# usamec/GAML

Measured on AMD Instinct MI355X. Metric: reads_per_sec_scored, higher is better.
Workload: dtype f64; 1 GPU; cfg3: 5 Mbp, 50x 2x150 paired, insert 300+-30; 833333 pairs in all, whole true genome as 1-2 walks, 8 rotating path sets, window cache warm; pairs_total=833333, pairs_per_gpu=833333, genome_bp=5000000, parallelism=reads sharded over 1 GPU(s)

## Files before the change

### gaml_amd/api.py

```python
from __future__ import annotations

import ctypes as C
import importlib.util
import os
import sys

import numpy as np

_HERE = os.path.dirname(os.path.abspath(__file__))
FLAVOUR = os.environ.get("GAML_HIP_FLAVOUR", "release")
LIB_PATH = os.environ.get("GAML_HIP_LIB") or os.path.join(_HERE, "libgaml_hip_dev.so" if FLAVOUR == "dev" else "libgaml_hip.so")

OK, EINVAL, ENODEVICE, EHIP, ESTATE = 0, -1, -2, -3, -4

_i32p = np.ctypeslib.ndpointer(np.int32, flags="C_CONTIGUOUS")
_i64p = np.ctypeslib.ndpointer(np.int64, flags="C_CONTIGUOUS")
_f64p = np.ctypeslib.ndpointer(np.float64, flags="C_CONTIGUOUS")
_u8p = np.ctypeslib.ndpointer(np.uint8, flags="C_CONTIGUOUS")

ALIGMENT = np.dtype([("position", np.int32), ("edit_dist", np.int32), ("read_id", np.int32), ("orientation", np.int32)])
PACBIO_ALIGMENT = np.dtype([("position", np.int32), ("position_end", np.int32), ("read_id", np.int32), ("pad_", np.int32),
                            ("logprob", np.float64)])


# ... 123 lines not shown
    L.gaml_hip_eval_coverage_finish_async.argtypes = [vp, C.c_int32, vp, C.c_int32, C.c_int32, vp]
    L.gaml_hip_eval_pacbio_pending.argtypes = [vp]
    L.gaml_hip_eval_pacbio_pending.restype = C.c_int32
    L.gaml_hip_eval_pacbio_intervals.argtypes = [vp, C.c_int32]
    L.gaml_hip_eval_pacbio_intervals.restype = C.c_int64
    L.gaml_hip_eval_pacbio_export_async.argtypes = [vp, C.c_int32, vp, C.c_int64, vp]
    L.gaml_hip_eval_pacbio_finish_async.argtypes = [vp, C.c_int32, vp, C.c_int64, C.c_int32, vp]
    L.gaml_hip_num_readsets.argtypes = [vp]
    L.gaml_hip_readset_kind.argtypes = [vp, C.c_int]
    L.gaml_hip_readset_reads.argtypes = [vp, C.c_int]
    L.gaml_hip_readset_reads.restype = C.c_int64
    L.gaml_hip_num_nodes.argtypes = [vp]
    L.gaml_hip_node_len.argtypes = [vp, C.c_int32]
    L.gaml_hip_read_probs.argtypes = [vp, C.c_int, _f64p, C.c_int64]
    L.gaml_hip_bad_bases.argtypes = [vp, C.c_int, C.POINTER(C.c_int64)]
    L.gaml_hip_window_count.argtypes = [vp, C.c_int, C.c_int]
    L.gaml_hip_window_count.restype = C.c_int64
    L.gaml_hip_window_records.argtypes = [vp, C.c_int, C.c_int, _i32p, C.c_int32, vp, C.c_int64]
    L.gaml_hip_window_records.restype = C.c_int64
    L.gaml_hip_align_window.argtypes = [vp, C.c_int, C.c_int, _i32p, C.c_int32]
    L.gaml_hip_align_window.restype = C.c_int64
    if hasattr(L, "gaml_hip_debug_prepare"):
        L.gaml_hip_debug_prepare.argtypes = [vp, _i32p, _i64p, C.c_int32]
    if hasattr(L, "gaml_hip_debug_occurrences"):
        L.gaml_hip_debug_occurrences.argtypes = [vp, C.c_int, C.c_int, _i32p, C.c_int64]
    if hasattr(L, "gaml_hip_debug_occurrences"):
        L.gaml_hip_debug_occurrences.restype = C.c_int64
    if hasattr(L, "gaml_hip_debug_table_occurrences"):
        L.gaml_hip_debug_table_occurrences.argtypes = [vp, C.c_int, C.c_int, _i32p, C.c_int64, _i64p]
    if hasattr(L, "gaml_hip_debug_table_occurrences"):
        L.gaml_hip_debug_table_occurrences.restype = C.c_int64
    if hasattr(L, "gaml_hip_debug_cov_layout"):
        L.gaml_hip_debug_cov_layout.argtypes = [vp, C.c_int, vp, C.c_int32, vp, vp, vp, C.c_int32, vp, C.c_int32, vp]
        L.gaml_hip_debug_cov_layout.restype = C.c_int32
    if hasattr(L, "gaml_hip_debug_window_walk"):
        L.gaml_hip_debug_window_walk.argtypes = [vp, C.c_int, C.c_int, C.c_int32, _i32p, C.c_int32]
    for new, old in (("gaml_hip_pair_classes", "gaml_hip_debug_class_counts"), ("gaml_hip_last_phases", "gaml_hip_debug_profile"),
                     ("gaml_hip_table_stats", "gaml_hip_debug_table_stats")):
        if not hasattr(L, new) and hasattr(L, old):
            setattr(L, new, getattr(L, old))
    L.gaml_hip_pair_classes.argtypes = [vp, C.c_int, _i64p]
    if hasattr(L, "gaml_hip_debug_fold_check"):
        L.gaml_hip_debug_fold_check.argtypes = [vp, C.c_int, _i64p]
    if hasattr(L, "gaml_hip_debug_radix_sort"):
        L.gaml_hip_debug_radix_sort.argtypes = [vp, C.c_void_p, C.c_void_p, C.c_int64, C.c_int, C.c_int, C.c_void_p]
    if hasattr(L, "gaml_hip_debug_tables_check"):
        L.gaml_hip_debug_tables_check.argtypes = [vp, C.c_int, _i64p]
    if hasattr(L, "gaml_hip_debug_static_check"):
        L.gaml_hip_debug_static_check.argtypes = [vp, C.c_int, _i64p]
    if hasattr(L, "gaml_hip_debug_set_knob"):
        L.gaml_hip_debug_set_knob.argtypes = [vp, C.c_int, C.c_int]
    if hasattr(L, "gaml_hip_debug_occ_route"):
        L.gaml_hip_debug_occ_route.argtypes = [vp, C.c_int, _i64p]
    if hasattr(L, "gaml_hip_debug_occ_check"):
        L.gaml_hip_debug_occ_check.argtypes = [vp, C.c_int, _i64p]
    if hasattr(L, "gaml_hip_debug_batch_bad_bases"):
        L.gaml_hip_debug_batch_bad_bases.argtypes = [vp, C.c_int, C.c_void_p, C.c_int32]
        L.gaml_hip_debug_batch_bad_bases.restype = C.c_int32
    if hasattr(L, "gaml_hip_shm_exchange_open"):
        L.gaml_hip_shm_exchange_open.argtypes = [vp, C.c_char_p, C.c_int32, C.c_int32, C.c_int32]
        L.gaml_hip_shm_allreduce_sum.argtypes = [vp, C.c_void_p, C.c_int32]
        L.gaml_hip_shm_exchange_close.argtypes = [vp, C.c_int32]
    if hasattr(L, "gaml_hip_fetch_async"):
        L.gaml_hip_fetch_async.argtypes = [vp, C.c_void_p, C.c_int32, C.c_void_p]
        L.gaml_hip_fetch_wait.argtypes = [vp, C.c_void_p, C.c_int32]
    if hasattr(L, "gaml_hip_advice_build"):
        L.gaml_hip_advice_build.argtypes = [vp, C.c_int, C.c_int32]
        L.gaml_hip_advice_index.argtypes = [vp, C.c_int, C.c_void_p, C.c_void_p, C.c_int64]
        L.gaml_hip_advice_index.restype = C.c_int64
        L.gaml_hip_advice_candidates.argtypes = [vp, C.c_int, _i32p, C.c_int32, _i32p, C.c_int32, C.c_int32, C.c_void_p, C.c_int64]
        L.gaml_hip_advice_candidates.restype = C.c_int64
    if hasattr(L, "gaml_hip_gap_profile"):
        L.gaml_hip_gap_profile.argtypes = [vp, _i32p, _i64p, C.c_int32, C.c_int32, C.c_int32, C.c_void_p, C.c_int32, C.c_void_p, C.c_void_p, C.c_void_p]
        L.gaml_hip_fix_gap_length.argtypes = [vp, _i32p, _i64p, C.c_int32, C.c_int32, C.c_int32, C.POINTER(C.c_int32), C.c_void_p, C.c_void_p,
                                              C.c_int32, C.POINTER(C.c_int32)]
        L.gaml_hip_gap_stats.argtypes = [vp, _i64p]
    if hasattr(L, "gaml_hip_debug_timeline"):
        L.gaml_hip_debug_timeline.argtypes = [vp, C.c_int, C.c_void_p, C.c_int64]
    L.gaml_hip_last_phases.argtypes = [vp, _f64p]
    L.gaml_hip_table_stats.argtypes = [vp, C.c_int, _i64p]
    L.gaml_hip_aligner_stats.argtypes = [vp, C.POINTER(C.c_int64), C.POINTER(C.c_int64), C.POINTER(C.c_double)]
    L.gaml_hip_aligner_stages.argtypes = [vp, _f64p]
    L.gaml_hip_last_timing.argtypes = [vp, _f64p]
    L.gaml_hip_set_event_timing.argtypes = [vp, C.c_int]
    L.gaml_hip_kernel_stats.argtypes = [vp, C.c_int, C.POINTER(C.c_int64), C.POINTER(C.c_double), C.POINTER(C.c_double)]
    return L


_lib = _load()

def lib():
    return _lib


def version() -> str:
    return _lib.gaml_hip_version().decode()


class FlatPaths:

    def __init__(self, paths):
        self.flat, self.offs = _flat(paths)
        self.n = len(paths)
        self.flat_ptr, self.offs_ptr = self.flat.ctypes.data, self.offs.ctypes.data

    def __len__(self):
# ... 475 lines not shown
        return {"full_rebuilds": int(out[0]), "delta_updates": int(out[1]), "dirty_pairs": int(out[2]), "worker_rebuilds": int(out[3]), "side_stream_rebuilds": int(out[3]),
                "batches_patched": int(out[4]), "batches_full": int(out[5]), "records_left_out": [int(out[6]), int(out[7])], "delta_records_left_out": int(out[8]),
                "static_index_pairs": int(out[9])}

    def aligner_stats(self):
        w, k, us = C.c_int64(), C.c_int64(), C.c_double()
        _lib.gaml_hip_aligner_stats(self._h, C.byref(w), C.byref(k), C.byref(us))
        return {"windows": w.value, "candidates": k.value, "us": us.value}

    def aligner_stages(self):
        out = np.zeros(6, np.float64)
        self._check(_lib.gaml_hip_aligner_stages(self._h, out))
        return {"strings_upload": out[0], "spans_candidates": out[1], "extension": out[2], "hits_d2h": out[3], "sort_file": out[4], "batches": int(out[5])}

    def last_phases(self):
        out = np.zeros(8, np.float64)
        _lib.gaml_hip_last_phases(self._h, out)
        return out

    def debug_timeline(self, rs: int, cap_waves: int = 1 << 16) -> np.ndarray:
        out = np.zeros((cap_waves, 8), np.uint64)
        n = self._check(_lib.gaml_hip_debug_timeline(self._h, rs, out.ctypes.data, cap_waves))
        return out[:n]

    def debug_set_knob(self, knob, value):
        self._check(_lib.gaml_hip_debug_set_knob(self._h, knob, value))

    def debug_fold_check(self, rs):
        out = np.zeros(6, np.int64)
        self._check(_lib.gaml_hip_debug_fold_check(self._h, rs, out))
        return {"records_left_out": [int(out[0]), int(out[1])], "compact_pairs": [int(out[2]), int(out[3])], "records_checked": int(out[4]),
                "violations": int(out[5])}

    def debug_radix_sort(self, keys, vals=None, begin_bit=0, end_bit=64, running_max=False):
        k = np.ascontiguousarray(keys, np.uint64).copy()
        v = None if vals is None else np.ascontiguousarray(vals, np.uint64).copy()
        m = np.zeros(len(k), np.uint64) if running_max else None
        self._check(_lib.gaml_hip_debug_radix_sort(self._h, k.ctypes.data, None if v is None else v.ctypes.data, len(k), begin_bit, end_bit,
                                                   None if m is None else m.ctypes.data))
        return k, v, m

    def debug_static_check(self, rs):
        out = np.zeros(8, np.int64)
        self._check(_lib.gaml_hip_debug_static_check(self._h, rs, out))
        return {"static_pairs": int(out[0]), "other_pairs": int(out[1]), "violations": int(out[2]), "no_record": int(out[3]),
                "different_windows": int(out[4]), "orientation": int(out[5]), "distance": int(out[6]), "edits_or_code": int(out[7])}

    def debug_occ_route(self, rs):
        out = np.zeros(6, np.int64)
        self._check(_lib.gaml_hip_debug_occ_route(self._h, rs, out))
        return {"device": int(out[0]), "host": int(out[1]), "fallbacks": int(out[2]), "compactions": int(out[3]),
                "pool_entries": int(out[4]), "shared_combinations": int(out[5])}

    def debug_occ_check(self, rs):
        out = np.zeros(4, np.int64)
        rc = _lib.gaml_hip_debug_occ_check(self._h, rs, out)
        res = {"compared": int(out[0]), "present": int(out[1]), "mismatches": int(out[2]), "lists": int(out[3])}
        if rc != 0 and res["compared"] == 0:
            self._check(rc)
        return res

    def debug_batch_bad_bases(self, rs):
        n = self._check(_lib.gaml_hip_debug_batch_bad_bases(self._h, rs, None, 0))
        out = np.zeros(max(1, n), np.int64)
        self._check(_lib.gaml_hip_debug_batch_bad_bases(self._h, rs, out.ctypes.data, n))
        return out[:n].tolist()

    def debug_tables_check(self, rs):
        out = np.zeros(8, np.int64)
        rc = _lib.gaml_hip_debug_tables_check(self._h, rs, out)
        res = {"pairs": int(out[0]), "compact": int(out[1]), "static": int(out[2]), "two": int(out[3]), "four": int(out[4]), "more": int(out[5]),
               "compared": int(out[6]), "mismatches": int(out[7])}
        if rc != 0 and res["compared"] == 0:
            self._check(rc)
        return res

    def debug_block_partials(self, rs, set_index=0):
        sums, zeros, lay = np.zeros(8192, np.float64), np.zeros(8192, np.int32), np.zeros(8, np.int32)
        _lib.gaml_hip_debug_block_partials.argtypes = [C.c_void_p, C.c_int, C.c_int32, _f64p, _i32p, C.c_int32, _i32p]
        n = _lib.gaml_hip_debug_block_partials(self._h, rs, set_index, sums, zeros, 8192, lay)
        return sums[:max(n, 0)].copy(), zeros[:max(n, 0)].copy(), lay.tolist()

    def pair_classes(self, rs):
        out = np.zeros(4, np.int64)
        self._check(_lib.gaml_hip_pair_classes(self._h, rs, out))
        return out

    debug_table_stats, debug_profile, debug_class_counts = table_stats, last_phases, pair_classes

    def last_timing(self):
        out = np.zeros(3, np.float64)
        _lib.gaml_hip_last_timing(self._h, out)
        return {"host_us": out[0], "device_wall_us": out[1], "kernel_us": out[2]}

    def set_event_timing(self, on):
        _lib.gaml_hip_set_event_timing(self._h, int(on))

    def kernel_stats(self, reset=False):
        n, us, b = C.c_int64(), C.c_double(), C.c_double()
        _lib.gaml_hip_kernel_stats(self._h, 1 if reset else 0, C.byref(n), C.byref(us), C.byref(b))
        return {"launches": n.value, "device_us": us.value, "algo_bytes": b.value}


def debug_sam_band(sam_line: str, total_len: int):
    raw = sam_line.encode()
    f = np.zeros(10, np.int32); r0 = np.zeros(1, np.int32)
# ... 20 lines not shown
```

### gaml_amd/csrc/ctx.hip.h

```cpp
#pragma once
#include <hip/hip_runtime.h>
#include <hip/hip_ext.h>
#include "radix_sort.hip.h"

#include <algorithm>
#include <atomic>
#include <fcntl.h>
#include <sys/mman.h>
#include <unistd.h>
#include <chrono>
#include <climits>
#include <limits>
#include <cmath>
#include <cstdio>
#include <cstdlib>
#include <cstring>
#include <immintrin.h>
#include <memory>
#include <set>
#include <string>
#include <thread>
#include <vector>

#include "aligner.hip.h"
// ... 229 lines not shown
  PairInfo pt;
  MateDev dev[2];
  TableDev tab;
  TableRebuild rebuild;
  BuildScratch scratch;
  BuildPlan build_plan;
  int64_t async_rebuilds = 0, retired_windows = 0, eval_count = 0;
  DevBuf lcode, len_combo_dev, combo_tabs, memo;
  int memo_codes = 0;
  bool statics_uploaded = false, kernels_warm = false, prereserved = false;
  DevBuf dl_slot, dl_spill, dl_rec[2], sp_rng[2], sp_rec[2], sp_slot, dstate;
  DevBuf dl_bins, dl_bin_count, dl_blk_tot, dl_wlist, dl_stamps;
  PinBuf h_dstate;
  size_t delta_cap = 0, cap_spill = 0, cap_sprec = 0;
  int64_t nd_est = 0, ns_est = 0;
  bool spill_may_grow = false;
  int dl_seq = 0;
  int64_t full_rebuilds = 0, delta_updates = 0;
  int quiet_calls = 0;
  int64_t delta_left_out = 0, delta_left_out_base = 0;
  bool compact_requested = false;
  PinBuf h_timeline; int timeline_waves = 0;
  PinBuf h_part_sum, h_part_zero;
  size_t host_part_stride = 0;
  int last_total_blocks = 0, last_sets = 1;
  int last_blocks[8] = {0, 0, 0, 0, 0, 0, 0, 0};
  bool last_host_partials = false;
  DevBuf probs, tabs, cov_bits, bad;
  DevBuf cov_multi;
  size_t cov_multi_used = 0;
  PinBuf h_bad;
  std::vector<int64_t> batch_bad;
  Arena arena;
  struct Persist {
    void* dev = nullptr; size_t bytes = 0;
    size_t cap_w[2] = {0, 0}, cap_lo[2] = {0, 0}, cap_m[2] = {0, 0};
    size_t off_tfloor = 0, off_occ[2] = {0, 0}, off_lo[2] = {0, 0}, off_m[2] = {0, 0};
    size_t cap_cov = 0, off_cov = 0;
    bool valid = false;
    size_t last_bytes = 0;
    void release() { if (dev) (void)hipFree(dev); dev = nullptr; bytes = 0; valid = false; }
  } persist;
  struct OccDev {
    DevBuf pool[2];
    size_t pool_cap[2] = {0, 0}, pool_used[2] = {0, 0};
    uint32_t pool_gen = 1;
    PinBuf stage;
    DevBuf tab[2][2], list[2][2];
    DevBuf stamp[2];
    size_t cap_w = 0, cap_list = 0;
    int32_t list_n[2][2] = {{0, 0}, {0, 0}};
    uint32_t serial = 0;
    PinBuf dup;
    bool taken = false;
    bool check_dup = false;
    bool image_stale = false;
    std::vector<std::vector<uint64_t>> shared;
    size_t shared_next = 0;
    std::vector<uint64_t> key;
    int64_t dev_calls = 0, host_calls = 0, fallbacks = 0, compactions = 0;
    void release() {
      for (int mt = 0; mt < 2; mt++) {
        pool[mt].release(); stamp[mt].release();
        for (int k = 0; k < 2; k++) { tab[mt][k].release(); list[mt][k].release(); }
      }
      stage.release(); dup.release();
    }
  } occdev;
  int64_t batches_patched = 0, batches_full = 0;
  size_t batch_slack = 0;
  hipEvent_t ev_tables = nullptr, ev_ovf = nullptr;
  PairedPlanner planner;
  OccImage image[2];
  std::vector<Occ> scratch_occ[2];
  Reducer red;
  Staging stage_pool;
  std::vector<double> ins_tab, floor_tab, logfloor_tab, covthr_tab;
  bool floor_positive = true;
  bool tabs_uploaded = false;
  int64_t last_bad_bases = 0;
  AdviceDev adv;
};

struct SingleSet {
  gaml_single_cfg cfg;
  ShortMate mate;
  ReadMajor rm;
  MateDev dev;
  DevBuf lens, probs, tabs, occ_arena;
  std::vector<Occ> last_occ;
  Reducer red;
  std::vector<double> floor_tab, logfloor_tab;
  bool tabs_uploaded = false;
  Staging stage;
};

struct DpDev {
  DevBuf path, jobs, ops, scratch, out, dbg;
  void release() { path.release(); jobs.release(); ops.release(); scratch.release(); out.release(); dbg.release(); }
};

struct PbSweepDev {
  DevBuf iv_off, iv;
  std::vector<int32_t> iv_off_host;
  uint64_t generation = ~0ull;
  DevBuf in, all;
  DevBuf key_begin, key_end, pos, key_begin_s, key_end_s, pos_s, end_max, tmp, bad;
  Staging stage;
  void release() {
    iv_off.release(); iv.release(); in.release(); all.release(); key_begin.release(); key_end.release(); pos.release();
    key_begin_s.release(); key_end_s.release(); pos_s.release(); end_max.release(); tmp.release(); bad.release();
    for (int k = 0; k < kRing; k++) { stage.host[k].release(); if (stage.done[k]) (void)hipEventDestroy(stage.done[k]); stage.done[k] = nullptr; stage.armed[k] = false; }
  }
};

struct PacbioSet {
// ... 8 lines not shown
  int64_t misses = 0;
  DevBuf d_lens, rec_off, rec_walk, rec_logp, walk_count, logprobs;
  Reducer red;
  int64_t last_bad_bases = 0;
  Staging stage;
  PbSweepDev sweep;
  bool have_reads = false;
  std::string bases;
  std::vector<int64_t> base_off;
  std::unordered_map<std::string, int32_t> name_id;
  DevBuf d_bases;
  DpDev dp;
  bool bases_uploaded = false;
  double dp_stats[8] = {0, 0, 0, 0, 0, 0, 0, 0};
};

struct PairedPrep {
  int64_t assembled_records = 0;
  std::vector<int32_t> slot_base, path_base, start_off, starts;
  int32_t total_bits = 0, n_paths = 0;
  bool general = false;
};

struct SetRef { int kind, idx; };

}
}

using namespace gaml;
using namespace gaml::detail;

struct gaml_hip_ctx {
  gaml::MultiState* multi = nullptr;
  gaml::CommState* comm = nullptr;
  int device = -1;
  DevBuf warm_buf; bool general_warm = false;
  AlnJob aln_job[2];
  hipStream_t stream = nullptr;
  hipStream_t aux_stream = nullptr;
  GraphStore g;
  bool have_graph = false;
  std::vector<std::unique_ptr<SingleSet>> singles;
  std::vector<std::unique_ptr<PairedSet>> paireds;
  std::vector<std::unique_ptr<PacbioSet>> pacbios;
  std::vector<SetRef> handles;
  int32_t rank = 0, world = 1;
  bool multi_shard = false;
  AlignScratch aln_scratch;
  AlignSmall aln_small[2];
  int64_t aln_windows = 0, aln_candidates = 0;
  double aln_us = 0;
  double aln_stage_us[5] = {0, 0, 0, 0, 0};
  int64_t aln_batches = 0;
  int knobs[24] = {0};
  bool direct_write = false;
  int32_t peers = 1;
  std::string err;
  bool event_timing = false;
  int event_every = 1;
  int64_t event_tick = 0;
  std::vector<std::pair<hipEvent_t, hipEvent_t>> ev_pool;
  std::vector<uint64_t> ev_call;
  uint64_t eval_serial = 0;
  size_t ev_used = 0;
  double t_host_us = 0, t_dev_wall_us = 0, t_kernel_us = 0;
  int64_t stat_launches = 0;
  double stat_device_us = 0, stat_algo_bytes = 0;
  DevBuf packed;
  PinBuf packed_host;
  char* shm_base = nullptr; size_t shm_bytes = 0; int shm_rank = 0, shm_world = 0, shm_cap = 0; unsigned long long shm_step = 0; std::string shm_name;
  PinBuf fetch_host;
  unsigned long long fetch_seq = 0;
  hipStream_t fetch_stream = nullptr;
  DevBuf batch_dev;
  PinBuf batch_host;
  int64_t gap_stats[4] = {0, 0, 0, 0};
  std::vector<int32_t> gap_flat;
  std::vector<int64_t> gap_offs;
  bool pending_open = false;
  std::vector<Walk> pending_paths;
  bool pending_paths_valid = false;
  int32_t pending_total_len = 0;
  std::vector<std::unique_ptr<PairedPrep>> pending_prep;
  double pending_host_us = 0;
  double prof[8] = {0, 0, 0, 0, 0, 0, 0, 0};
  bool used_default_stream = false;
  double* status_dst = nullptr; double status_a = 0, status_b = 0; bool status_done = false;
  bool host_results = false;
  bool occ_route = false;
  bool defer_cov = false;
  struct PendingCov { int paired_idx; CovArgs args; double* out4; };
  std::vector<PendingCov> pending_cov;
  struct PendingPacbio {
    int pacbio_idx;
    double* out4;
    int32_t n_paths;
    int64_t n_node, n_own;
  };
  std::vector<PendingPacbio> pending_pb;
};
```

### gaml_amd/csrc/debug_api.hip.h

```cpp
#pragma once

int gaml_hip_debug_prepare(gaml_hip_ctx* c, const int32_t* flat, const int64_t* offs, int32_t n_paths) {
  if (!c || n_paths < 0 || (n_paths > 0 && (!flat || !offs))) return fail(c, GAML_HIP_EINVAL, "bad arguments");
  if (c->multi) {
    for (int k = 0; k < gaml::multi_num_shards(c->multi); k++)
      if (int e = gaml_hip_debug_prepare(gaml::multi_shard(c->multi, k), flat, offs, n_paths)) return fail(c, e, gaml_hip_last_error(gaml::multi_shard(c->multi, k)));
    return GAML_HIP_OK;
  }
  if (!c->have_graph) return fail(c, GAML_HIP_ESTATE, "no graph set");
  std::vector<Walk> paths = unflatten(flat, offs, n_paths);
  for (auto& h : scoring_order(c)) {
    if (h.kind == 0) { std::vector<Occ> occs; prepare_single_host(c, *c->singles[h.idx], paths, occs); }
    else if (h.kind == 1) {
      PairedPrep p;
      PairedSet& ps = *c->paireds[h.idx];
      if (int e = prepare_paired_structure(c, ps, flat, offs, n_paths)) return e;
      if (int e = align_pending_pair(c, ps)) return e;
      if (int e = prepare_paired_tables_host(c, ps, p)) return e;
    }
  }
  if (c->peers == 1) {
    for (ShortMate* m : filter_mates(c)) m->unsynced.clear();
  }
  return GAML_HIP_OK;
// ... 28 lines not shown
  for (Occ& o : v) { auto it = pos.find(o.path); o.path = it == pos.end() ? -1 : it->second; }
  std::sort(v.begin(), v.end(), [](const Occ& a, const Occ& b) { return a.path != b.path ? a.path < b.path : (a.rank != b.rank ? a.rank < b.rank : a.wid < b.wid); });
  for (int64_t i = 0; i < (int64_t)v.size() && i < cap; i++) {
    const Occ& o = v[(size_t)i];
    out5[5 * i] = o.wid; out5[5 * i + 1] = o.shift; out5[5 * i + 2] = o.min_pos; out5[5 * i + 3] = o.path; out5[5 * i + 4] = o.rank;
  }
  return (int64_t)v.size();
}

int32_t gaml_hip_debug_cov_layout(gaml_hip_ctx* c, int rs, int32_t* slot_base, int32_t cap_slots, int32_t* path_base, int32_t* start_off, int32_t* slots,
                                   int32_t cap_paths, int32_t* starts, int32_t cap_starts, int32_t* counts4) {
  MULTI_SHARD0(c);
  if (!c || rs < 0 || rs >= (int)c->handles.size() || c->handles[rs].kind != 1) return -1;
  PairedSet& ps = *c->paireds[c->handles[rs].idx];
  if (!(ps.cfg.penalty_constant > 0) || ps.planner.full_calls + ps.planner.incremental_calls == 0) return -1;
  struct { std::vector<int32_t> slot_base, path_base, start_off, starts, slots; } L;
  {
    PairedPrep p;
    paired_cov_build(ps, true, p);
    L.slot_base.swap(p.slot_base); L.path_base.swap(p.path_base); L.start_off.swap(p.start_off); L.starts.swap(p.starts);
    L.slots = ps.planner.slots();
  }
  const int32_t n = (int32_t)L.slots.size();
  if (counts4) { counts4[0] = (int32_t)L.slot_base.size(); counts4[1] = n; counts4[2] = (int32_t)L.starts.size(); counts4[3] = L.path_base.back(); }
  for (int32_t k = 0; k < (int32_t)L.slot_base.size() && k < cap_slots; k++) slot_base[k] = L.slot_base[k];
  for (int32_t k = 0; k <= n && k <= cap_paths && cap_paths > 0; k++) { path_base[k] = L.path_base[k]; start_off[k] = L.start_off[k]; }
  for (int32_t k = 0; k < n && k < cap_paths; k++) slots[k] = L.slots[k];
  for (int32_t k = 0; k < (int32_t)L.starts.size() && k < cap_starts; k++) starts[k] = L.starts[k];
  return n;
}

int32_t gaml_hip_debug_window_walk(gaml_hip_ctx* c, int rs, int mate, int32_t wid, int32_t* out, int32_t cap) {
  MULTI_SHARD0(c);
  ShortMate* m = mate_of(c, rs, mate);
  if (!m || wid < 0 || wid >= (int32_t)m->win_walk.size()) return -1;
  const Walk& w = *m->win_walk[wid];
  for (int32_t i = 0; i < (int32_t)w.size() && i < cap; i++) out[i] = w[i];
  return (int32_t)w.size();
}



int gaml_hip_debug_timeline(gaml_hip_ctx* c, int rs, unsigned long long* out, int64_t cap_waves) {
  MULTI_SHARD0(c);
  if (!c || rs < 0 || rs >= (int)c->handles.size() || c->handles[rs].kind != 1 || !out) return fail(c, GAML_HIP_EINVAL, "bad arguments");
  PairedSet& s = *c->paireds[c->handles[rs].idx];
  if (!s.h_timeline.p) return 0;
  const int64_t n = std::min<int64_t>(cap_waves, s.timeline_waves);
  memcpy(out, s.h_timeline.p, (size_t)n * 8 * sizeof(unsigned long long));
  return (int)n;
}

int gaml_hip_debug_set_knob(gaml_hip_ctx* c, int knob, int value) {
  if (!c || knob < 0 || knob >= 24) return GAML_HIP_EINVAL;
  if (c->multi) { for (int k = 0; k < gaml::multi_num_shards(c->multi); k++) gaml::multi_shard(c->multi, k)->knobs[knob] = value; return GAML_HIP_OK; }
  c->knobs[knob] = value;
  return GAML_HIP_OK;
}


static void paired_base_records(const PairTables& pt, int32_t slot, int mt, std::vector<RecQuad>& out) {
  const int64_t n0s = pt.class_count[0];
  if (slot < n0s) {
    const uint64_t r = pt.rec8[mt][slot];
    if (r != kNoRec8) out.push_back(RecQuad{(int32_t)(r & 0xffffff), (int32_t)((r >> 24) & 0xfffffff), (int32_t)((r >> 52) & 63) | ((int32_t)((r >> 58) & 1) << 8), 0});
  } else {
    const RecQuad& f = pt.rm[mt].first[slot - n0s];
    if (f.wid >= 0) {
      const int cnt1 = 1 + (int)((uint32_t)f.flags >> 9);
      for (int q = 0; q < cnt1; q++) { RecQuad r = q == 0 ? f : pt.rm[mt].extra[f.link + q - 1]; r.flags &= 0x1ff; r.link = 0; out.push_back(r); }
    }
  }
}

int gaml_hip_debug_fold_check(gaml_hip_ctx* c, int rs, int64_t* out6) {
  MULTI_SHARD0(c);
  if (!c || rs < 0 || rs >= (int)c->handles.size() || c->handles[rs].kind != 1 || !out6) return fail(c, GAML_HIP_EINVAL, "bad arguments");
  PairedSet& s = *c->paireds[c->handles[rs].idx];
  for (int mt = 0; mt < 2; mt++) for (const Window& w : s.mate[mt].wins) if (w.first < 0 && w.count > 0) return fail(c, GAML_HIP_ESTATE, "host-only check: some windows' records exist in the device pool only (use gaml_hip_debug_tables_check)");
  PairTables with, without;
  build_pair_tables(s.mate[0], s.mate[1], with, true);
  build_pair_tables(s.mate[0], s.mate[1], without, false);
  int64_t checked = 0, bad = 0;
  const int64_t n = s.mate[0].n_local();
  std::vector<RecQuad> a, b;
  for (int mt = 0; mt < 2; mt++) {
    const ShortMate& m = s.mate[mt];
    for (int64_t read = 0; read < n; read++) {
      a.clear(); b.clear();
      paired_base_records(with, with.slot_of_read[read], mt, a);
      paired_base_records(without, without.slot_of_read[read], mt, b);
      size_t ia = 0;
      for (size_t ib = 0; ib < b.size(); ib++) {
        checked++;
        const RecQuad& r = b[ib];
        if (ia < a.size() && a[ia].wid == r.wid && a[ia].pos == r.pos && a[ia].flags == r.flags) { ia++; continue; }
        const Window& j = m.wins[r.wid];
        bool ok = false;
        if (j.head >= 0) {
          auto it = m.solo_of_node.find(j.head);
          if (it != m.solo_of_node.end() && m.wins[it->second].active)
            for (size_t q = 0; q < b.size(); q++) ok = ok || (b[q].wid == it->second && b[q].pos == r.pos);
        }
        bad += !ok;
      }
      bad += ia != a.size();
    }
// ... 122 lines not shown
    for (Window& w : hm[mt].wins) if (w.dfirst < 0) { w.count = 0; }
  }
  PairTables pt;
  build_pair_tables(hm[0], hm[1], pt, KNOB(c, 16) != 1, paired_static_ins_n(c, s));
  const int64_t n = s.mate[0].n_local();
  int64_t compared = 0, bad = 0;
  auto fetch = [&](const DevBuf& d, size_t bytes, std::vector<char>& out) -> int {
    out.resize(bytes);
    if (bytes) HIP_TRY(c, hipMemcpy(out.data(), d.p, bytes, hipMemcpyDeviceToHost));
    return 0;
  };
  auto cmp = [&](const DevBuf& d, const void* host, size_t bytes, size_t elem, const char* what) -> int {
    std::vector<char> v;
    if (int e = fetch(d, bytes, v)) return e;
    int64_t b0 = bad;
    for (size_t k = 0; k < bytes / elem; k++) { compared++; if (memcmp(v.data() + k * elem, (const char*)host + k * elem, elem) != 0) bad++; }
    if (bad != b0 && getenv("GAML_HIP_TRACE_HOST")) fprintf(stderr, "tables_check: %s differs in %lld of %zu entries\n", what, (long long)(bad - b0), bytes / elem);
    return 0;
  };
  for (int k = 0; k < 4; k++) { compared++; bad += T.class_count[k] != pt.class_count[k]; }
  compared++; bad += T.n0a != pt.n0a;
  if (bad == 0) {
    const int64_t n0 = pt.class_count[0], n16 = n - n0;
    if (int e = cmp(T.slot_of_read, pt.slot_of_read.data(), (size_t)n * 4, 4, "slot_of_read")) return e;
    if (int e = cmp(T.read_of_slot, pt.read_of_slot.data(), (size_t)n * 4, 4, "read_of_slot")) return e;
    for (int mt = 0; mt < 2; mt++) {
      if (int e = cmp(T.rec8[mt], pt.rec8[mt].data(), (size_t)n0 * 8, 8, "rec8")) return e;
      if (int e = cmp(T.first[mt], pt.rm[mt].first.data(), (size_t)n16 * 16, 16, "first")) return e;
      if (int e = cmp(T.extra[mt], pt.rm[mt].extra.data(), pt.rm[mt].extra.size() * 16, 16, "extra")) return e;
      if (int e = cmp(T.inl[mt], pt.inl[mt].data(), pt.inl[mt].size() * 16, 16, "inl")) return e;
      compared++; bad += T.extras[mt] != (int64_t)pt.rm[mt].extra.size();
      compared++; bad += T.dropped[mt] != pt.dropped_records[mt];
    }
    if (int e = cmp(T.len_code, pt.len_code.data(), (size_t)n0, 1, "len_code")) return e;
    if (int e = cmp(T.static_idx, pt.static_idx.data(), (size_t)pt.n0a * 4, 4, "static_idx")) return e;
    if (int e = cmp(T.len12, pt.len12.data(), (size_t)n16 * 4, 4, "len12")) return e;
    compared++; bad += pt.len_combo != s.pt.len_combo;
  }
  out8[0] = n; out8[1] = T.class_count[0]; out8[2] = T.n0a; out8[3] = T.class_count[1]; out8[4] = T.class_count[2]; out8[5] = T.class_count[3];
  out8[6] = compared; out8[7] = bad;
  T.release();
  return bad ? fail(c, GAML_HIP_ESTATE, "record tables: the device build differs from the host restatement") : GAML_HIP_OK;
}

int gaml_hip_debug_occ_route(gaml_hip_ctx* c, int rs, int64_t* out6) {
  MULTI_SHARD0(c);
  if (!c || !out6 || rs < 0 || rs >= (int)c->handles.size() || c->handles[rs].kind != 1) return fail(c, GAML_HIP_EINVAL, "bad arguments");
  const PairedSet::OccDev& D = c->paireds[c->handles[rs].idx]->occdev;
  out6[0] = D.dev_calls; out6[1] = D.host_calls; out6[2] = D.fallbacks; out6[3] = D.compactions;
  out6[4] = (int64_t)(D.pool_used[0] + D.pool_used[1]); out6[5] = (int64_t)D.shared.size();
  return GAML_HIP_OK;
}

int gaml_hip_debug_occ_check(gaml_hip_ctx* c, int rs, int64_t* out4) {
  MULTI_SHARD0(c);
  if (!c || !out4 || rs < 0 || rs >= (int)c->handles.size() || c->handles[rs].kind != 1) return fail(c, GAML_HIP_EINVAL, "bad arguments");
  PairedSet& ps = *c->paireds[c->handles[rs].idx];
  const PairedSet::OccDev& D = ps.occdev;
  out4[0] = out4[1] = out4[2] = out4[3] = 0;
  if (!D.image_stale) return GAML_HIP_OK;
  HIP_TRY(c, hipSetDevice(c->device));
  HIP_TRY(c, hipStreamSynchronize(c->stream));
  const PlanView& v = ps.planner.view();
  for (int mt = 0; mt < 2; mt++) {
    OccImage im;
    im.build(ps.mate[mt].wins.size(), v, mt);
    const size_t n = im.occ12.size();
    std::vector<Occ12> dev(n);
    if (n) HIP_TRY(c, hipMemcpy(dev.data(), occdev_table(ps, mt), n * sizeof(Occ12), hipMemcpyDeviceToHost));
    for (size_t w = 0; w < n; w++) {
      const Occ12& h = im.occ12[w];
      const Occ12& d = dev[w];
      const bool absent = h.lo == ~0u && h.hi == ~0u;
      out4[0]++;
      if (!absent) out4[1]++;
      if (absent ? (d.lo != ~0u || d.hi != ~0u) : (d.lo != h.lo || d.hi != h.hi || d.rank != h.rank)) out4[2]++;
    }
    if (!im.general_wids.empty()) out4[3]++;
  }
  if (out4[2] || out4[3]) return fail(c, GAML_HIP_ESTATE, "device occurrence tables differ from the host image");
  return GAML_HIP_OK;
}

int32_t gaml_hip_debug_batch_bad_bases(gaml_hip_ctx* c, int rs, int64_t* out, int32_t cap) {
  MULTI_SHARD0(c);
  if (!c || rs < 0 || rs >= (int)c->handles.size() || c->handles[rs].kind != 1 || cap < 0 || (cap > 0 && !out)) return fail(c, GAML_HIP_EINVAL, "bad arguments");
  const std::vector<int64_t>& b = c->paireds[c->handles[rs].idx]->batch_bad;
  for (size_t k = 0; k < b.size() && k < (size_t)cap; k++) out[k] = b[k];
  return (int32_t)b.size();
}
```

### gaml_amd/csrc/host_model.cc

```cpp
#include "host_model.h"

#include <algorithm>
#include <chrono>
#include <cmath>
#include <cstdlib>
#include <cstring>
#include <fstream>
#include <thread>

namespace gaml {

void GraphStore::finish() {
  norm.resize(n());
  std::unordered_map<std::string, int32_t> tiny;
  for (int32_t i = 0; i < n(); i++) {
    norm[i] = i;
    if (len(i) > 3) continue;
    std::string s(seq(i), len(i));
    auto it = tiny.find(s);
    if (it == tiny.end()) tiny.emplace(s, i);
    else norm[i] = it->second;
  }
}

// ... 895 lines not shown
    for (int32_t k = 0; k < n_paths; k++) {
      const int32_t id = cur_ids_[k];
      if (!redo[id]) continue;
      if (!is_new_[k]) {
        const PathMemo& pm = *memos_[id];
        removed_.push_back(Removed{cur_slots_[k], {pm.assembled[0], pm.assembled[1]}, {pm.occ[0], pm.occ[1]}});
      }
      work_.push_back(k);
    }
    std::vector<int32_t> keep;
    for (int32_t sid : stale_) if (sid < (int32_t)memos_.size() && memos_[sid]->use_count > 0 && (!memos_[sid]->valid[0] || !memos_[sid]->valid[1])) keep.push_back(sid);
    stale_.swap(keep);
  }
  const int64_t total = n_paths > 0 ? offs[n_paths] - base : 0;
  prev_flat_.assign(flat + base, flat + base + total);
  prev_offs_.resize((size_t)n_paths + 1);
  for (int32_t k = 0; k <= n_paths; k++) prev_offs_[k] = (n_paths > 0 ? offs[k] : 0) - base;
  have_prev_ = true;
  return true;
}

static void occ_prepack(const std::vector<Occ>& occ, std::vector<OccPre>& pre) {
  pre.resize(occ.size());
  for (size_t k = 0; k < occ.size(); k++) {
    const Occ& o = occ[k];
    const int32_t mp = o.min_pos < -32768 ? -32768 : o.min_pos;
    pre[k] = OccPre{o.min_pos <= 32767 ? o.wid : ~o.wid, (uint32_t)o.shift, (uint32_t)(uint16_t)(int16_t)mp, o.rank};
  }
}

static bool occ_pre_plain(const std::vector<OccPre>& pre) {
  std::vector<int32_t> w(pre.size());
  for (size_t k = 0; k < pre.size(); k++) { if (pre[k].wid < 0) return false; w[k] = pre[k].wid; }
  std::sort(w.begin(), w.end());
  return std::adjacent_find(w.begin(), w.end()) == w.end();
}

void PairedPlanner::invalidate_thresholds() {
  for (auto& pm : memos_) pm->occ_valid[0] = pm->occ_valid[1] = false;
  have_prev_ = false;
}

void PairedPlanner::finish(ShortMate mate[2]) {
  auto redo_occ = [&](PathMemo& pm) {
    for (int mt = 0; mt < 2; mt++) {
      if (pm.occ_valid[mt]) continue;
      pm.occ[mt].clear();
      occurrences_from_placements(mate[mt], pm.pl[mt], pm.occ[mt]);
      pm.assembled[mt] = 0;
      for (const Occ& o : pm.occ[mt]) pm.assembled[mt] += mate[mt].wins[o.wid].count;
      occ_prepack(pm.occ[mt], pm.pre[mt]);
      pm.pre_plain[mt] = occ_pre_plain(pm.pre[mt]);
      pm.dev_off[mt] = -1;
      pm.occ_valid[mt] = true;
    }
  };
  if (!incremental_) {
    for (int32_t id : cur_ids_) redo_occ(*memos_[id]);
    assembled_[0] = assembled_[1] = 0;
    for (int32_t id : cur_ids_) { assembled_[0] += memos_[id]->assembled[0]; assembled_[1] += memos_[id]->assembled[1]; }
  } else {
    for (int32_t k : work_) redo_occ(*memos_[cur_ids_[k]]);
  }
}

const PlanView& PairedPlanner::view() {
  if (!view_valid_) {
    view_.paths.clear();
    for (int32_t id : cur_ids_) view_.paths.push_back(memos_[id].get());
    view_valid_ = true;
  }
  return view_;
}

void PairedPlanner::apply(ShortMate mate[2], OccImage image[2], bool build_image, bool image_stale) {
  if (!incremental_) {
    const PlanView& v = view();
    for (int32_t id : cur_ids_) {
      PathMemo& pm = *memos_[id];
      if (pm.touched_serial == retire_serial_) continue;
      for (int mt = 0; mt < 2; mt++) for (const Occ& o : pm.occ[mt]) mate[mt].touch(o.wid);
      pm.touched_serial = retire_serial_;
    }
    if (build_image) for (int mt = 0; mt < 2; mt++) image[mt].build(mate[mt].wins.size(), v, mt);
    return;
  }
  if (image_stale) {
    for (int mt = 0; mt < 2; mt++) {
      for (const Removed& r : removed_) assembled_[mt] -= r.assembled[mt];
      for (int32_t k : work_) assembled_[mt] += memos_[cur_ids_[k]]->assembled[mt];
    }
    for (int32_t id : cur_ids_) {
      PathMemo& pm = *memos_[id];
      if (pm.touched_serial == retire_serial_) continue;
      for (int mt = 0; mt < 2; mt++) for (const Occ& o : pm.occ[mt]) mate[mt].touch(o.wid);
      pm.touched_serial = retire_serial_;
    }
    rebuild_images(mate, image);
    return;
  }
  for (int32_t k : work_) {
    PathMemo& pm = *memos_[cur_ids_[k]];
    if (pm.touched_serial == retire_serial_) continue;
    for (int mt = 0; mt < 2; mt++) for (const Occ& o : pm.occ[mt]) mate[mt].touch(o.wid);
    pm.touched_serial = retire_serial_;
  }
// ... 681 lines not shown
```

### gaml_amd/csrc/host_model.h

```cpp
#pragma once
#include <climits>
#include <cstdint>
#include <memory>
#include <string>
#include <unordered_map>
#include <vector>

#include "../../include/gaml_hip.h"

namespace gaml {

constexpr int kTail = 300;
constexpr int kSeed = 15;

struct GraphStore {
  std::string bases;
  std::vector<int64_t> off;
  std::vector<int32_t> norm;
  int32_t n() const { return (int32_t)off.size() - 1; }
  int32_t len(int32_t node) const { return (int32_t)(off[node + 1] - off[node]); }
  const char* seq(int32_t node) const { return bases.data() + off[node]; }
  void finish();
  bool load_lastgraph(const std::string& file, std::string* err);
};
// ... 157 lines not shown
struct OccTable {
  std::vector<OccQuad> direct;
  std::vector<int32_t> multi_off;
  std::vector<OccQuad> multi;
};
void build_occ_table(size_t n_windows, const std::vector<Occ>& occs, OccTable& out);

void split_contigs(const Walk& path, std::vector<std::pair<int32_t, int32_t>>& ctg_ranges, std::vector<int32_t>& gaps);

struct PlanView;
struct Occ12 { uint32_t lo, hi; int32_t rank; };
struct OccImage {
  std::vector<Occ12> occ12;
  std::vector<int32_t> multi_off;
  std::vector<OccQuad> multi;
  std::vector<int32_t> general_wids;
  void build(size_t n_windows, const PlanView& view, int mate, const std::vector<int32_t>* slots = nullptr,
             const std::vector<int32_t>* pos_of_slot = nullptr);
  void add_path(size_t n_windows, const std::vector<Occ>& occ, int32_t slot);
  void remove_path(const std::vector<Occ>& occ, int32_t slot);
  void finalize(const std::vector<int32_t>& pos_of_slot);
  std::vector<int32_t> changed;
  bool changed_all = true, lists_changed = true;
  void dump(std::vector<Occ>& out) const;
  template <class F> void for_each_present(F f) const { for (int32_t w : touched_) if (cnt_[w] > 0) f(w); }
  void take_changed() { changed.clear(); changed_all = false; lists_changed = false; if (++mark_serial_ == 0) { std::fill(mark_.begin(), mark_.end(), 0); mark_serial_ = 1; } }
 private:
  void grow(size_t n_windows);
  void mark(int32_t w) { if (mark_[w] != mark_serial_) { mark_[w] = mark_serial_; changed.push_back(w); } }
  void set_direct(int32_t w, const OccQuad& q);
  std::vector<int32_t> touched_, stale_, cnt_, list_of_;
  std::vector<uint32_t> stamp_, mark_;
  uint32_t serial_ = 0, mark_serial_ = 1;
  struct Pending { int32_t wid; OccQuad q; };
  std::vector<Pending> pending_;
  std::unordered_map<int32_t, std::vector<OccQuad>> gen_;
  bool lists_dirty_ = false;
};

struct OccPre { int32_t wid; uint32_t lo, hi; int32_t rank; };

struct PathMemo {
  Walk path;
  bool registered[2] = {false, false};
  bool first_pending[2] = {false, false};
  bool valid[2] = {false, false};
  bool occ_valid[2] = {false, false};
  std::vector<Placement> pl[2];
  std::vector<Occ> occ[2];
  std::vector<OccPre> pre[2];
  bool pre_plain[2] = {false, false};
  int64_t dev_off[2] = {-1, -1};
  uint32_t dev_gen[2] = {0, 0};
  int64_t assembled[2] = {0, 0};
  std::vector<int32_t> starts;
  int32_t length = 0;
  int32_t first_idx = -1, first_end = -1;
  int32_t final_last_end = -2;
  int32_t use_count = 0;
  uint32_t touched_serial = 0;
  uint64_t last_used = 0;
  uint32_t serial = 0;
};

struct PlanView {
  std::vector<const PathMemo*> paths;
};

class PairedPlanner {
 public:
  bool begin(const GraphStore& g, ShortMate mate[2], const int32_t* flat, const int64_t* offs, int32_t n_paths,
             bool allow_incremental, std::string* err);
  void finish(ShortMate mate[2]);
  void apply(ShortMate mate[2], OccImage image[2], bool build_image = true, bool image_stale = false);
  void rebuild_images(ShortMate mate[2], OccImage image[2]);
  const std::vector<int32_t>& ids() const { return cur_ids_; }
  PathMemo& memo(int32_t id) { return *memos_[id]; }
  void mark_used(ShortMate mate[2], const OccImage image[2]);
  void note_rebuild(bool retired_some) { rebuild_clock_ = clock_; if (retired_some) retire_serial_++; }
  void invalidate_thresholds();
  void forget_previous() { have_prev_ = false; }
  const PlanView& view();
  void flat_occurrences(int mate, std::vector<Occ>& out);
  size_t memo_count() const { return memos_.size(); }
  int32_t total_len() const { return total_len_; }
  int64_t assembled(int mate) const { return assembled_[mate]; }
  int32_t n_paths() const { return (int32_t)cur_ids_.size(); }
  bool last_was_incremental() const { return incremental_; }
  const std::vector<int32_t>& slots() const { return cur_slots_; }
  int32_t slot_count() const { return next_slot_; }
  uint64_t hits = 0, misses = 0, incremental_calls = 0, full_calls = 0;
 private:
  int32_t lookup_or_create(const GraphStore& g, const int32_t* p, int32_t len, std::string* err);
  void drain(ShortMate mate[2]);
  void build_placements(const GraphStore& g, ShortMate& m, int mt, PathMemo& pm, int32_t id);
  void registration_chain(const GraphStore& g, ShortMate mate[2], int32_t from, int32_t to);
  std::vector<std::unique_ptr<PathMemo>> memos_;
  std::unordered_map<Walk, int32_t, WalkHasher> by_path_;
  std::unordered_map<Walk, std::vector<std::pair<int32_t, uint32_t>>, WalkHasher> missed_[2];
  PlanView view_;
  bool view_valid_ = false;
  std::vector<int32_t> cur_ids_;
  std::vector<int32_t> cur_slots_;
  std::vector<int32_t> free_slots_, pos_of_slot_;
  int32_t next_slot_ = 0;
  std::vector<int32_t> prev_flat_;
// ... 42 lines not shown
```

### gaml_amd/csrc/kernels.hip.h

```cpp
#pragma once
#include <hip/hip_runtime.h>
#include <stdint.h>

namespace gaml {

constexpr int kBlock = 256;
constexpr int kMaxBlocks = 2048;
enum { kDsDirty = 0, kDsSpill = 1, kDsTop0 = 2, kDsTop1 = 3, kDsOverflow = 4, kDsSeq = 5, kDsInts = 8 };

__device__ __forceinline__ unsigned long long occ8_of(const Occ12* t, unsigned w) { const Occ12* e = t + w; return (unsigned long long)e->lo | ((unsigned long long)e->hi << 32); }

struct MateView {
  const int4* first;
  const int4* extra;
  const int4* occ;
  const Occ12* occ12;
  const int* multi_off;
  const int4* multi;
  const double* mism_pow;
  const double* match_pow;
};

struct PairedArgs {
  int total_blocks, blocks0a, n0a, n_codes;
  int blocks0;
  int blocks01, blocks012;
  int main_blocks;
  const double2* memo;
  uint32_t* cov_bits;
  const unsigned long long* rec8[2];
  const double2* static_val;
  const Occ12* occ12[2];
  double* probs;
  double* part_sum;
  int* part_zero;
  double log_two_T;
  double tfloor0, logfloor0;
  uint32_t len_combo0; int pad0_;
  MateView m[2];
  const uint32_t* len12;
  const double* ins_tab;
  int ins_n;
  const double* floor_tab;
  const double* logfloor_tab;
  const double* covthr_tab;
  double two_T;
  int n;
  const int* path_base;
  double covthr0;
  const unsigned char* len_code;
  const uint32_t* len_combo;
  const double* pe[2];
  const double* floor_c;
  const double* logfloor_c;
  const double* covthr_c;
  int lt_codes;
  const double* tfloor_c;
  const int4* inl[2];
  int n0;
  const int* static_idx;
  int n01;
  int n_main;
  unsigned long long* timeline;
  const int* dstate;
  const int* dirty_slots;
  const int4* dirty_recs[2];
  const int* dirty_spill;
  const int2* spill_rng[2];
  const int4* spill_recs[2];
  const int* spill_slot;
  unsigned* ticket;
  double* out;
  double n_reads;
  double* status_out;
  double status_a, status_b;
};

struct Cand { int path, pos, edit, orient, rank, k; bool valid; };

__device__ __forceinline__ int4 occ_from_compact(unsigned long long o, int rk) {
  const int4 e = make_int4((int)(unsigned)o, (int)(short)(o >> 32), (int)((o >> 48) & 0x7fff), rk);
  return o == ~0ull ? make_int4(0, 0, -1, 0) : e;
}
__device__ __forceinline__ int4 mate_occ(const MateView& v, int w) {
  if (v.occ) return v.occ[w];
  const Occ12 e = v.occ12[w];
  return occ_from_compact((unsigned long long)e.lo | ((unsigned long long)e.hi << 32), e.rank);
}

__device__ __forceinline__ Cand make_cand(const int4& r, const int4& o, int k) {
  Cand c;
  c.path = o.z; c.pos = r.y + o.x; c.edit = r.z & 0xff; c.orient = (r.z >> 8) & 1;
  c.rank = o.w; c.k = k; c.valid = r.y >= o.y;
  return c;
}

struct TableSrc {
  const MateView* v;
  int4 r0;
  __device__ __forceinline__ int count() const { return r0.x < 0 ? 0 : 1 + (int)((unsigned)r0.z >> 9); }
  __device__ __forceinline__ int4 get(int k) const { return k == 0 ? r0 : v->extra[r0.w + k - 1]; }
};
struct ListSrc {
  const int4* recs;
  int cnt;
  __device__ __forceinline__ int count() const { return cnt; }
  __device__ __forceinline__ int4 get(int k) const { return recs[k]; }
};

template <class Src, class F>
__device__ __forceinline__ void for_each_cand_src(const MateView& v, const Src& src, F f) {
  const int cnt = src.count();
  for (int k = 0; k < cnt; k++) {
    int4 r = src.get(k);
    if (r.x < 0) continue;
    int4 o = mate_occ(v, r.x);
    if (o.z < 0) continue;
    if (o.w >= 0) {
      f(make_cand(r, o, k));
    } else {
      const int s = -o.w - 1;
      for (int q = v.multi_off[s]; q < v.multi_off[s + 1]; q++) f(make_cand(r, v.multi[q], k));
    }
  }
}
template <class F>
__device__ __forceinline__ void for_each_cand(const MateView& v, const int4& r0, F f) {
  for_each_cand_src(v, TableSrc{&v, r0}, f);
}
// ... 107 lines not shown

constexpr int kTicketWords = 17;
__device__ __forceinline__ void grid_finish(double s, int z, int my_slot, int n_partials, double* part_sum, int* part_zero,
                                            unsigned* ticket, double* out, double bad_bases, double n_reads, double* sh_s, int* sh_z,
                                            double* status_out = nullptr, double status_a = 0.0, double status_b = 0.0) {
  __shared__ bool is_last;
  if (threadIdx.x == 0) {
    __hip_atomic_store(&part_sum[my_slot], s, __ATOMIC_RELAXED, __HIP_MEMORY_SCOPE_AGENT);
    __hip_atomic_store(&part_zero[my_slot], z, __ATOMIC_RELAXED, __HIP_MEMORY_SCOPE_AGENT);
    asm volatile("s_waitcnt vmcnt(0)" ::: "memory");
    const int g = my_slot & 15;
    const unsigned in_group = (unsigned)((n_partials - g + 15) >> 4), groups = (unsigned)min(16, n_partials);
    bool last = false;
    if (__hip_atomic_fetch_add(&ticket[1 + g], 1u, __ATOMIC_RELAXED, __HIP_MEMORY_SCOPE_AGENT) == in_group - 1)
      last = __hip_atomic_fetch_add(&ticket[0], 1u, __ATOMIC_RELAXED, __HIP_MEMORY_SCOPE_AGENT) == groups - 1;
    is_last = last;
  }
  __syncthreads();
  if (!is_last) return;
  double ts = 0; int tz = 0;
  for (int b = threadIdx.x; b < n_partials; b += kBlock) {
    ts += __hip_atomic_load(&part_sum[b], __ATOMIC_RELAXED, __HIP_MEMORY_SCOPE_AGENT);
    tz += __hip_atomic_load(&part_zero[b], __ATOMIC_RELAXED, __HIP_MEMORY_SCOPE_AGENT);
  }
  __syncthreads();
  block_reduce(ts, tz, sh_s, sh_z);
  if (threadIdx.x < kTicketWords) __hip_atomic_store(&ticket[threadIdx.x], 0u, __ATOMIC_RELAXED, __HIP_MEMORY_SCOPE_AGENT);
  if (threadIdx.x == 0) {
    out[0] = ts;
    out[1] = (double)tz;
    if (bad_bases >= 0) out[2] = bad_bases;
    out[3] = n_reads;
    if (status_out) { status_out[0] = status_a; status_out[1] = status_b; }
  }
}

struct PairVal { double t, logt; int key, kind; };

__device__ __forceinline__ void finish_read(const PairedArgs& a, int i, double acc, int L1, int L2, double& lsum, int& zeros, PairVal* cap = nullptr) {
  if (cap) *cap = PairVal{acc, 0.0, L1 + L2, 3};
  a.probs[i] = acc;
  const double p = acc / a.two_T;
  const int s = L1 + L2;
  if (p < a.floor_tab[s]) { zeros++; lsum += a.logfloor_tab[s]; }
  else lsum += log(p);
}

template <int K>
struct RegCands {
  int path[K], pos[K], ef[K], rank[K];
  bool valid[K], live[K];
};

template <int K>
__device__ __forceinline__ bool cands_from_records(const MateView& v, const int4 (&r)[K], RegCands<K>& c) {
  int4 o[K];
  bool multi = false;
  Occ12 e[K];
#pragma unroll
  for (int k = 0; k < K; k++) e[k] = v.occ12[r[k].x >= 0 ? r[k].x : 0];
#pragma unroll
  for (int k = 0; k < K; k++) o[k] = occ_from_compact((unsigned long long)e[k].lo | ((unsigned long long)e[k].hi << 32), e[k].rank);
#pragma unroll
  for (int k = 0; k < K; k++) if (r[k].x < 0) o[k] = make_int4(0, 0, -1, 0);
#pragma unroll
  for (int k = 0; k < K; k++) {
    multi |= (o[k].z >= 0 && o[k].w < 0);
    c.path[k] = o[k].z; c.pos[k] = r[k].y + o[k].x; c.ef[k] = r[k].z & 0x1ff; c.rank[k] = o[k].w;
    c.valid[k] = r[k].x >= 0 && o[k].z >= 0 && r[k].y >= o[k].y;
  }
#pragma unroll
  for (int i = 0; i < K; i++) {
    bool lv = c.valid[i];
#pragma unroll
    for (int j = 0; j < K; j++)
      if (j != i) lv = lv && !(c.valid[j] && c.path[j] == c.path[i] && c.pos[j] == c.pos[i] &&
                               (c.rank[j] > c.rank[i] || (c.rank[j] == c.rank[i] && j > i)));
    c.live[i] = lv;
  }
  return multi;
}
template <int K>
__device__ __forceinline__ bool load_cands_inline(const MateView& v, const int4* rec, RegCands<K>& c) {
  int4 r[K];
#pragma unroll
  for (int k = 0; k < K; k++) r[k] = rec[k];
  return cands_from_records<K>(v, r, c);
}

template <int K>
__device__ __forceinline__ double score_regs(const PairedArgs& a, const RegCands<K>& c1, const RegCands<K>& c2, int L1, int L2) {
  int n1 = 0, n2 = 0;
  Cand x, y;
  x.path = -1; x.pos = 0; x.edit = 0; x.orient = 0; y = x;
#pragma unroll
  for (int i = 0; i < K; i++) {
    if (c1.live[i]) { n1++; x.path = c1.path[i]; x.pos = c1.pos[i]; x.edit = c1.ef[i] & 0xff; x.orient = c1.ef[i] >> 8; }
    if (c2.live[i]) { n2++; y.path = c2.path[i]; y.pos = c2.pos[i]; y.edit = c2.ef[i] & 0xff; y.orient = c2.ef[i] >> 8; }
  }
  if (n1 == 0 || n2 == 0) return 0.0;
  if (n1 == 1 && n2 == 1) return x.path == y.path ? pair_term(a, x, y, L1, L2) : 0.0;
  double acc = 0.0;
#pragma unroll
  for (int i = 0; i < K; i++) {
#pragma unroll
    for (int j = 0; j < K; j++) {
      if (c1.live[i] && c2.live[j] && c1.path[i] == c2.path[j]) {
        Cand x, y;
        x.path = c1.path[i]; x.pos = c1.pos[i]; x.edit = c1.ef[i] & 0xff; x.orient = c1.ef[i] >> 8;
        y.path = c2.path[j]; y.pos = c2.pos[j]; y.edit = c2.ef[j] & 0xff; y.orient = c2.ef[j] >> 8;
        acc += pair_term(a, x, y, L1, L2);
      }
    }
// ... 144 lines not shown

__device__ __forceinline__ void compact_finish(const PairedArgs& a, int i, const Compact1& c, const CompactPrep& q, double2 m,
                                               double& lsum, int& zeros, PairVal* cap = nullptr) {
  if (q.memo_idx >= 0) {
    const double t = m.x;
    if (cap) *cap = PairVal{t, m.y, c.lc, 1};
    compact_cover(a, c, q, t);
    __builtin_nontemporal_store(t, &a.probs[i]);
    const bool floored = t < a.tfloor_c[c.lc];
    lsum += floored ? a.logfloor_c[c.lc] : m.y - a.log_two_T;
    zeros += (int)floored;
    return;
  }
  double t = 0.0;
  if (q.scores) { t = compact_term_tables(a, c, q); compact_cover(a, c, q, t); }
  finish_read_compact(a, i, t, c.lc, lsum, zeros, cap);
}

__device__ __forceinline__ void finish_val(const PairedArgs& a, int i, const PairVal& v, bool store, double& lsum, int& zeros) {
  if (v.kind == 0) return;
  if (store) __builtin_nontemporal_store(v.t, &a.probs[i]);
  if (v.kind == 1) {
    const bool floored = v.t < a.tfloor_c[v.key];
    lsum += floored ? a.logfloor_c[v.key] : v.logt - a.log_two_T;
    zeros += (int)floored;
  } else if (v.kind == 2) {
    if (v.t == 0.0 && a.floor_c[v.key] > 0.0) { zeros++; lsum += a.logfloor_c[v.key]; return; }
    const double p = v.t / a.two_T;
    if (p < a.floor_c[v.key]) { zeros++; lsum += a.logfloor_c[v.key]; }
    else lsum += log(p);
  } else {
    const double p = v.t / a.two_T;
    if (p < a.floor_tab[v.key]) { zeros++; lsum += a.logfloor_tab[v.key]; }
    else lsum += log(p);
  }
}

__device__ __forceinline__ void compact_load(const PairedArgs& a, int i, bool ok, Compact1& c) {
  c.r1 = ok ? a.rec8[0][i] : kNone8;
  c.r2 = ok ? a.rec8[1][i] : kNone8;
  c.lc = ok ? a.len_code[i] : 0;
}

#if defined(GAML_HIP_DEV) && defined(GAML_GEN_X)
#define GAML_GEN_OFF(bit) ((GAML_GEN_X) & (bit))
#else
#define GAML_GEN_OFF(bit) 0
#endif
struct SlotRange { int lo, hi, lb, blocks; };
__device__ __forceinline__ SlotRange compact_range(const PairedArgs& a, int lb) {
  return lb < a.blocks0a ? SlotRange{0, a.n0a, lb, a.blocks0a} : SlotRange{a.n0a, a.n0, lb - a.blocks0a, a.blocks0 - a.blocks0a};
}

template <bool GEN>
__device__ __forceinline__ void paired_compact_body(const PairedArgs& a, const SlotRange rg, double& lsum, int& zeros) {
  const int stride = rg.blocks * kBlock, hi = rg.hi;
  int i0 = rg.lo + rg.lb * kBlock + threadIdx.x;
  if (i0 >= hi) return;
  Compact1 c0, c1;
  compact_load(a, i0, true, c0);
  compact_load(a, i0 + stride, i0 + stride < hi, c1);
  while (true) {
    const int i1 = i0 + stride;
    const bool two = i1 < hi;
    const int j0 = i0 + 2 * stride;
    const bool more = j0 < hi;
    Compact1 n0v, n1v;
    compact_load(a, j0, more, n0v);
    compact_load(a, j0 + stride, j0 + stride < hi, n1v);
    const uint32_t l0 = a.len_combo[c0.lc], l1 = a.len_combo[c1.lc];
    c0.L1 = l0 & 0xffff; c0.L2 = l0 >> 16; c1.L1 = l1 & 0xffff; c1.L2 = l1 >> 16;
    const bool d0 = c0.r1 == kDirty8, d1 = c1.r1 == kDirty8;
    if (d0) { c0.r1 = kNone8; c0.r2 = kNone8; }
    if (d1) { c1.r1 = kNone8; c1.r2 = kNone8; }
    c0.o1 = c0.r1 != kNone8 ? occ8_of(a.occ12[0], (unsigned)(c0.r1 & 0xffffff)) : kNone8;
    c0.o2 = c0.r2 != kNone8 ? occ8_of(a.occ12[1], (unsigned)(c0.r2 & 0xffffff)) : kNone8;
    c1.o1 = c1.r1 != kNone8 ? occ8_of(a.occ12[0], (unsigned)(c1.r1 & 0xffffff)) : kNone8;
    c1.o2 = c1.r2 != kNone8 ? occ8_of(a.occ12[1], (unsigned)(c1.r2 & 0xffffff)) : kNone8;
    CompactPrep q0, q1;
    compact_prep(a, c0, q0);
    compact_prep(a, c1, q1);
    const double2 m0 = q0.memo_idx >= 0 ? a.memo[q0.memo_idx] : make_double2(0.0, 0.0);
    const double2 m1 = q1.memo_idx >= 0 ? a.memo[q1.memo_idx] : make_double2(0.0, 0.0);
    if (!d0 && !q0.skip) compact_finish(a, i0, c0, q0, m0, lsum, zeros);
    else if (GEN && q0.skip) { const GenOut o = compact_general_call(kernel_args_address(), i0, -1); lsum += o.add; zeros += o.zeros; }
    if (two && !d1 && !q1.skip) compact_finish(a, i1, c1, q1, m1, lsum, zeros);
    else if (GEN && two && q1.skip) { const GenOut o = compact_general_call(kernel_args_address(), i1, -1); lsum += o.add; zeros += o.zeros; }
    if (!more) break;
    c0 = n0v; c1 = n1v;
    i0 = j0;
  }
}

constexpr int kPairZero = -1, kPairOther = -(1 << 20);
__device__ __forceinline__ void cover_marks(const PairedArgs& a, uint2 r1, uint2 r2, uint2 o1, uint2 o2) {
  const int p1 = (int)(__funnelshift_r(r1.x, r1.y, 24) & 0xfffffffu), p2 = (int)(__funnelshift_r(r2.x, r2.y, 24) & 0xfffffffu);
  const int x = p1 + (int)o1.x, y = p2 + (int)o2.x;
  const int base = a.path_base[(o1.y >> 16) & 0x7fffu];
  mark_bit(a.cov_bits, base + max(x, y));
  mark_bit(a.cov_bits, base + min(x, y));
}
__device__ __forceinline__ void cover_marks_set(uint32_t* bits, const int* slot_base, uint2 r1, uint2 r2, uint2 o1, uint2 o2) {
  const int p1 = (int)(__funnelshift_r(r1.x, r1.y, 24) & 0xfffffffu), p2 = (int)(__funnelshift_r(r2.x, r2.y, 24) & 0xfffffffu);
  const int x = p1 + (int)o1.x, y = p2 + (int)o2.x;
  const int base = slot_base[(o1.y >> 16) & 0x7fffu];
  mark_bit(bits, base + max(x, y));
  mark_bit(bits, base + min(x, y));
}
__device__ __forceinline__ int compact_state(const PairedArgs& a, uint2 r1, uint2 r2, uint2 o1, uint2 o2, unsigned lc, uint32_t l12,
                                             bool in_range, bool& skip) {
  const bool v1 = r1.y != ~0u, v2 = r2.y != ~0u;
  const bool w1 = v1 & (o1.y != ~0u), w2 = v2 & (o2.y != ~0u);
  const bool here = in_range & !(r1.y == ~0u && r1.x == 0xfffffffeu);
  skip = here & ((w1 & ((int)o1.y < 0)) | (w2 & ((int)o2.y < 0)));
  const int L1 = l12 & 0xffff, L2 = l12 >> 16;
  const int p1 = (int)(__funnelshift_r(r1.x, r1.y, 24) & 0xfffffffu), p2 = (int)(__funnelshift_r(r2.x, r2.y, 24) & 0xfffffffu);
  const int x = p1 + (int)o1.x, y = p2 + (int)o2.x;
  const unsigned or1 = (r1.y >> 26) & 1u, or2 = (r2.y >> 26) & 1u;
  const bool fwd = x < y;
  const int dist = fwd ? y - x + L2 : x - y + L1;
  const bool scores = w1 & w2 & !skip & (((o1.y ^ o2.y) >> 16) == 0)
                      & (p1 >= (int)(short)(o1.y & 0xffffu)) & (p2 >= (int)(short)(o2.y & 0xffffu))
                      & (or1 != or2) & (or1 == (fwd ? 0u : 1u));
  const unsigned e1 = (r1.y >> 20) & 63u, e2 = (r2.y >> 20) & 63u;
  const bool in_memo = scores & ((unsigned)dist < (unsigned)a.ins_n) & (lc < (unsigned)a.lt_codes) & (e1 < 7u) & (e2 < 7u);
  const int idx = (int)((lc * 7u + e1) * 7u + e2) * a.ins_n + dist;
  int state = in_memo ? idx : ((skip | scores) ? kPairOther : kPairZero - (int)lc);
  if (!here) state = kPairOther - 1;
  return state;
}

template <bool GEN, bool TL = false, bool ONE = false, bool COV = false>
__device__ __forceinline__ void paired_compact4_body(const PairedArgs& a, const SlotRange rg, double& lsum, int& zeros) {
  const unsigned stride = (unsigned)rg.blocks * kBlock, n0 = (unsigned)rg.hi;
  unsigned long long* tl = TL ? a.timeline + ((size_t)blockIdx.x * (kBlock / 64) + (threadIdx.x >> 6)) * 8 : nullptr;
#define GAML_STAMP(slot, dep) if (TL) { asm volatile("s_waitcnt vmcnt(0)" ::: "memory"); if ((threadIdx.x & 63) == 0) tl[slot] = (unsigned long long)wall_clock64() + ((dep) == 0x12345u ? 1 : 0); }
  const char* const rec0 = (const char*)a.rec8[0];
  const char* const rec1 = (const char*)a.rec8[1];
  const char* const occ0 = (const char*)a.occ12[0];
  const char* const occ1 = (const char*)a.occ12[1];
  const char* const memo = (const char*)a.memo;
  char* const probs = (char*)a.probs;
  const uint32_t l12_one = ONE ? a.len_combo[0] : 0u;
  const double logfloor_one = ONE ? a.logfloor_c[0] : 0.0, tfloor_one = ONE ? a.tfloor_c[0] : 0.0, log2T = a.log_two_T;
  const double covthr_one = COV && ONE ? a.covthr0 : 0.0;
  for (unsigned base = (unsigned)rg.lo + (unsigned)rg.lb * kBlock + threadIdx.x; base < n0; base += 4 * stride) {
    uint2 r1[4], r2[4], o1[4], o2[4];
    unsigned lc[4];
#pragma unroll
    for (int k = 0; k < 4; k++) {
      const unsigned ic = base + k * stride < n0 ? base + k * stride : base;
      r1[k] = *(const uint2*)(rec0 + ic * 8u); r2[k] = *(const uint2*)(rec1 + ic * 8u); lc[k] = ONE ? 0u : (unsigned)a.len_code[ic];
    }
    GAML_STAMP(2, r1[0].x ^ r1[1].x ^ r1[2].x ^ r1[3].x ^ r2[0].x ^ r2[3].x)
#pragma unroll
    for (int k = 0; k < 4; k++) {
      const Occ12* e1 = (const Occ12*)(occ0 + (r1[k].y != ~0u ? (r1[k].x & 0xffffffu) : 0u) * 12u);
      const Occ12* e2 = (const Occ12*)(occ1 + (r2[k].y != ~0u ? (r2[k].x & 0xffffffu) : 0u) * 12u);
      o1[k] = make_uint2(e1->lo, e1->hi); o2[k] = make_uint2(e2->lo, e2->hi);
    }
    GAML_STAMP(3, o1[0].x ^ o1[1].x ^ o1[2].x ^ o1[3].x ^ o2[0].x ^ o2[3].x)
    int state[4];
    unsigned skip_bits = 0;
#pragma unroll
    for (int k = 0; k < 4; k++) {
      bool skip;
      state[k] = compact_state(a, r1[k], r2[k], o1[k], o2[k], lc[k], ONE ? l12_one : a.len_combo[lc[k]], base + k * stride < n0, skip);
      skip_bits |= (unsigned)skip << k;
    }
    double2 m[4];
#pragma unroll
    for (int k = 0; k < 4; k++) m[k] = *(const double2*)(memo + (unsigned)max(state[k], 0) * 16u);
    GAML_STAMP(4, (unsigned)(__double2loint(m[0].x) ^ __double2loint(m[1].x) ^ __double2loint(m[2].x) ^ __double2loint(m[3].x)))
    bool other = false;
    unsigned mark_bits = 0;
#pragma unroll
    for (int k = 0; k < 4; k++) {
      double* const out = (double*)(probs + (base + k * stride) * 8u);
      if (state[k] >= 0) {
        if (COV) mark_bits |= (unsigned)(m[k].x > (ONE ? covthr_one : a.covthr_c[lc[k]])) << k;
        __builtin_nontemporal_store(m[k].x, out);
        const bool floored = m[k].x < (ONE ? tfloor_one : a.tfloor_c[lc[k]]);
        lsum += floored ? (ONE ? logfloor_one : a.logfloor_c[lc[k]]) : m[k].y - log2T;
        zeros += (int)floored;
      } else if (state[k] > kPairOther) {
        __builtin_nontemporal_store(0.0, out);
        zeros++;
        lsum += ONE ? logfloor_one : a.logfloor_c[kPairZero - state[k]];
      } else other |= state[k] == kPairOther && !((skip_bits >> k) & 1u);
    }
    if (COV) {
#pragma unroll
      for (int k = 0; k < 4; k++)
        if ((mark_bits >> k) & 1u) cover_marks(a, r1[k], r2[k], o1[k], o2[k]);
    }
    GAML_STAMP(5, 0u)
    if (__any(other)) {
#pragma unroll 1
      for (int k = 0; k < 4; k++) {
        if (state[k] != kPairOther || ((skip_bits >> k) & 1u)) continue;
        const int i = (int)(base + k * stride);
        Compact1 d;
        compact_load(a, i, true, d);
        d.o1 = d.r1 != kNone8 ? occ8_of(a.occ12[0], (unsigned)(d.r1 & 0xffffff)) : kNone8;
        d.o2 = d.r2 != kNone8 ? occ8_of(a.occ12[1], (unsigned)(d.r2 & 0xffffff)) : kNone8;
        const uint32_t l = a.len_combo[d.lc];
        d.L1 = l & 0xffff; d.L2 = l >> 16;
        CompactPrep q;
        compact_prep(a, d, q);
        compact_finish(a, i, d, q, make_double2(0.0, 0.0), lsum, zeros);
      }
    }
    if (GEN && !GAML_GEN_OFF(8) && __any(skip_bits != 0)) {
#pragma unroll 1
      for (int k = 0; k < 4; k++)
        if ((skip_bits >> k) & 1u) { const GenOut o = compact_general_call(kernel_args_address(), (int)(base + k * stride), -1); lsum += o.add; zeros += o.zeros; }
    }
  }
#undef GAML_STAMP
}

#ifndef GAML_LEAN_ENTRY
#define GAML_LEAN_ENTRY 1
#endif
#if GAML_LEAN_ENTRY && defined(__HIP_DEVICE_COMPILE__)
#define GAML_FRESH_ARGS(name, fallback)                                                                                   \
  const __attribute__((address_space(4))) PairedArgs* name##_p =                                                          \
      (const __attribute__((address_space(4))) PairedArgs*)__builtin_amdgcn_kernarg_segment_ptr();                        \
  asm volatile("" : "+s"(name##_p));                                                                                      \
  const PairedArgs name = *name##_p;
#else
#define GAML_FRESH_ARGS(name, fallback) const PairedArgs& name = fallback;
#endif
#ifndef GAML_STATIC_P
#define GAML_STATIC_P 4
#endif
#ifndef GAML_STATIC_PIPE
#define GAML_STATIC_PIPE 0
#endif
#if defined(GAML_HIP_DEV) && defined(GAML_STATIC_X)
#define GAML_TIMING_X(bit) ((GAML_STATIC_X) & (bit))
#else
#define GAML_TIMING_X(bit) 0
#endif
__global__ __launch_bounds__(kBlock) void static_values_kernel(const int* static_idx, int n0a, const double2* memo, double2* static_val) {
  for (int i = blockIdx.x * kBlock + threadIdx.x; i < n0a; i += gridDim.x * kBlock) {
    const int mi = static_idx[i];
    static_val[i] = mi >= 0 ? memo[mi] : make_double2(0.0, 0.0);
  }
}

template <bool GEN, bool TL = false, bool ONE = false, bool COV = false>
__device__ __forceinline__ void paired_static4_body(const PairedArgs& a, const SlotRange rg, double& lsum, int& zeros) {
  constexpr int P = GAML_STATIC_P;
  const unsigned stride = (unsigned)rg.blocks * kBlock, n0 = (unsigned)rg.hi;
  unsigned long long* tl = TL ? a.timeline + ((size_t)blockIdx.x * (kBlock / 64) + (threadIdx.x >> 6)) * 8 : nullptr;
#define GAML_STAMP(slot, dep) if (TL && first_round) { asm volatile("s_waitcnt vmcnt(0)" ::: "memory"); if ((threadIdx.x & 63) == 0) tl[slot] = (unsigned long long)wall_clock64() + ((dep) == 0x12345u ? 1 : 0); }
  const char* const rec0 = (const char*)a.rec8[0];
  const char* const rec1 = (const char*)a.rec8[1];
  const char* const sval = (const char*)a.static_val;
  const char* const occ0 = (const char*)a.occ12[0];
  const char* const occ1 = (const char*)a.occ12[1];
  char* const probs = (char*)a.probs;
  const double logfloor_one = ONE ? a.logfloor0 : 0.0, tfloor_one = ONE ? a.tfloor0 : 0.0, log2T = a.log_two_T;
  const double covthr_one = COV && ONE ? a.covthr0 : 0.0;
  unsigned base = (unsigned)rg.lo + (unsigned)rg.lb * kBlock + threadIdx.x;
  if (base >= n0) return;
  uint2 r1[P], r2[P];
  double2 m[P];
  unsigned lc[P];
#pragma unroll
  for (int k = 0; k < P; k++) {
    const unsigned ic = base + k * stride < n0 ? base + k * stride : base;
    r1[k] = *(const uint2*)(rec0 + ic * 8u); r2[k] = *(const uint2*)(rec1 + ic * 8u); m[k] = GAML_TIMING_X(4) ? make_double2(1e-9 * (double)ic, -20.0) : *(const double2*)(sval + ic * 16u);
    lc[k] = ONE ? 0u : (unsigned)a.len_code[ic];
  }
  bool first_round = true;
  while (true) {
    GAML_STAMP(2, r1[0].x ^ r2[0].x ^ (unsigned)__double2loint(m[0].x))
    uint2 o1[P], o2[P];
#pragma unroll
    for (int k = 0; k < P; k++) {
      const unsigned w1 = (r1[k].x & 0xffffffu) & (0u - (unsigned)(r1[k].y != ~0u)), w2 = (r2[k].x & 0xffffffu) & (0u - (unsigned)(r2[k].y != ~0u));
      const Occ12* e1 = (const Occ12*)(occ0 + w1 * 12u);
      const Occ12* e2 = (const Occ12*)(occ1 + w2 * 12u);
      o1[k] = make_uint2(e1->lo, e1->hi); o2[k] = make_uint2(e2->lo, e2->hi);
      if (GAML_TIMING_X(1)) { o1[k] = make_uint2(r1[k].x >> 8, 0u); o2[k] = make_uint2(r1[k].x >> 8, 0u); }
    }
    const unsigned nbase = base + P * stride;
    const bool more = nbase < n0;
    uint2 nr1[P], nr2[P];
    double2 nm[P];
    unsigned nlc[P];
    if (GAML_STATIC_PIPE && __any(more)) {
#pragma unroll
      for (int k = 0; k < P; k++) {
        const unsigned ic = nbase + k * stride < n0 ? nbase + k * stride : base;
        nr1[k] = *(const uint2*)(rec0 + ic * 8u); nr2[k] = *(const uint2*)(rec1 + ic * 8u); nm[k] = *(const double2*)(sval + ic * 16u);
        nlc[k] = ONE ? 0u : (unsigned)a.len_code[ic];
      }
    }
    GAML_STAMP(3, o1[0].x ^ o2[0].x)
    GAML_STAMP(4, 0u)
    unsigned skip_bits = 0, mark_bits = 0;
#pragma unroll
    for (int k = 0; k < P; k++) {
      const bool none1 = r1[k].y == ~0u, none2 = r2[k].y == ~0u;
      const bool here = (base + k * stride < n0) & !(none1 & (r1[k].x == 0xfffffffeu));
      const bool w1 = !none1 & (o1[k].y != ~0u), w2 = !none2 & (o2[k].y != ~0u);
      const bool gen = here & ((w1 & ((int)o1[k].y < 0)) | (w2 & ((int)o2[k].y < 0)));
      const bool same = (o1[k].x == o2[k].x) & (((o1[k].y ^ o2[k].y) >> 16) == 0);
      const int p1 = (int)(__funnelshift_r(r1[k].x, r1[k].y, 24) & 0xfffffffu), p2 = (int)(__funnelshift_r(r2[k].x, r2[k].y, 24) & 0xfffffffu);
      const bool kept = (p1 >= (int)(short)(o1[k].y & 0xffffu)) & (p2 >= (int)(short)(o2[k].y & 0xffffu));
      const bool both = here & !gen & w1 & w2;
      const bool scores = both & same & kept;
      const bool poison = both & !same;
      const bool counted = here & !gen;
      skip_bits |= (unsigned)gen << k;
      const double t = scores ? m[k].x : 0.0;
      const bool floored = counted & (!scores | (t < (ONE ? tfloor_one : a.tfloor_c[lc[k]])));
      const double lf = ONE ? logfloor_one : a.logfloor_c[lc[k]];
      double add = floored ? lf : m[k].y - log2T;
      add = counted ? add : 0.0;
      add = poison ? __builtin_nan("") : add;
      lsum += add;
      zeros += (int)floored;
      if (counted && !GAML_TIMING_X(2)) __builtin_nontemporal_store(t, (double*)(probs + (base + k * stride) * 8u));
      if (COV) mark_bits |= (unsigned)(scores & (t > (ONE ? covthr_one : a.covthr_c[lc[k]]))) << k;
    }
    if (COV) {
#pragma unroll
      for (int k = 0; k < P; k++)
        if ((mark_bits >> k) & 1u) cover_marks(a, r1[k], r2[k], o1[k], o2[k]);
    }
    if (GEN && !GAML_GEN_OFF(1) && __any(skip_bits != 0)) {
#pragma unroll 1
      for (int k = 0; k < P; k++)
        if ((skip_bits >> k) & 1u) { const GenOut o = compact_general_call(kernel_args_address(), (int)(base + k * stride), -1); lsum += o.add; zeros += o.zeros; }
    }
    GAML_STAMP(5, 0u)
    first_round = false;
    if (!more) break;
    base = nbase;
    if (GAML_STATIC_PIPE) {
#pragma unroll
      for (int k = 0; k < P; k++) { r1[k] = nr1[k]; r2[k] = nr2[k]; m[k] = nm[k]; lc[k] = nlc[k]; }
    } else {
#pragma unroll
      for (int k = 0; k < P; k++) {
        const unsigned ic = base + k * stride < n0 ? base + k * stride : base;
        r1[k] = *(const uint2*)(rec0 + ic * 8u); r2[k] = *(const uint2*)(rec1 + ic * 8u); m[k] = GAML_TIMING_X(4) ? make_double2(1e-9 * (double)ic, -20.0) : *(const double2*)(sval + ic * 16u);
        lc[k] = ONE ? 0u : (unsigned)a.len_code[ic];
      }
    }
  }
#undef GAML_STAMP
}

#ifndef GAML_GEN_CANDS
#define GAML_GEN_CANDS 32
#endif
constexpr int kGenCands = GAML_GEN_CANDS;
#ifdef GAML_GEN_STAMPS
__device__ unsigned long long g_gen_stamp[32];
#define GEN_STAMP(k) do { asm volatile("s_waitcnt vmcnt(0) lgkmcnt(0)" ::: "memory"); const unsigned long long now_ = wall_clock64(); \
  if (__ffsll((long long)__ballot(1)) - 1 == (int)(threadIdx.x & 63)) atomicAdd(&g_gen_stamp[k], now_ - gen_t_); atomicMax(&g_gen_stamp[16 + k], now_ - gen_t_); if (now_ - gen_t_ > 1000) atomicAdd(&g_gen_stamp[24 + k], 1ull); gen_t_ = now_; } while (0)
#define GEN_STAMP_BEGIN unsigned long long gen_t_ = wall_clock64(); const unsigned long long gen_t0_ = gen_t_; if (__ffsll((long long)__ballot(1)) - 1 == (int)(threadIdx.x & 63)) atomicAdd(&g_gen_stamp[15], 1ull);
#else
#define GEN_STAMP(k) do { } while (0)
#define GEN_STAMP_BEGIN
#endif
constexpr int kGenListBatch = 8;
template <int K>
__device__ __forceinline__ bool general_pair_staged(const PairedArgs& a, const int4 (&r1)[K], const int4 (&r2)[K], int L1, int L2, double& acc_out, int4* cand) {
  int n[2] = {0, 0};
  unsigned live[2] = {0, 0};
  Occ12 e[2][K];
  int lb[2][K], le[2][K];
  GEN_STAMP_BEGIN
#pragma unroll
  for (int m = 0; m < 2; m++)
#pragma unroll
    for (int k = 0; k < K; k++) { const int4& r = m == 0 ? r1[k] : r2[k]; e[m][k] = a.m[m].occ12[r.x >= 0 ? r.x : 0]; }
  GEN_STAMP(0);
#pragma unroll
  for (int m = 0; m < 2; m++)
#pragma unroll
    for (int k = 0; k < K; k++) {
      const int4& r = m == 0 ? r1[k] : r2[k];
      const bool occurs = r.x >= 0 && !(e[m][k].lo == ~0u && e[m][k].hi == ~0u);
      const bool list = occurs && e[m][k].rank < 0;
      lb[m][k] = le[m][k] = 0;
      if (list) { const int s = -e[m][k].rank - 1; lb[m][k] = a.m[m].multi_off[s]; le[m][k] = a.m[m].multi_off[s + 1]; }
      else if (occurs) le[m][k] = -1;
    }
  GEN_STAMP(1);
  bool fits = true;
#pragma unroll
  for (int m = 0; m < 2; m++) {
    int4* const cm = cand + m * kGenCands;
#pragma unroll
    for (int k = 0; k < K; k++) {
      const int4& r = m == 0 ? r1[k] : r2[k];
      const bool single = le[m][k] == -1;
      const int cnt = single ? 1 : le[m][k] - lb[m][k];
      if (!__any(cnt > 0)) continue;
      if (n[m] + cnt > kGenCands) fits = false;
      const int4 one = occ_from_compact((unsigned long long)e[m][k].lo | ((unsigned long long)e[m][k].hi << 32), e[m][k].rank);
// ... 50 lines not shown
  return true;
}
constexpr int kOvfCap = 128;
constexpr int kGenWaveSlots = 2 * kOvfCap / (2 * kGenCands);
__device__ __forceinline__ int4* gen_wave_slot(int4* wave_lds, bool mine) {
  const unsigned long long m = __ballot(mine);
  const int rank = __popcll(m & ((1ull << (threadIdx.x & 63)) - 1ull));
  return (wave_lds && mine && rank < kGenWaveSlots) ? wave_lds + rank * 2 * kGenCands : nullptr;
}

template <int K>
__device__ __forceinline__ void score_cands_and_finish(const PairedArgs& a, int i, uint32_t l12, const RegCands<K>& x, const RegCands<K>& y,
                                                       double& lsum, int& zeros, PairVal* cap = nullptr) {
  const int L1 = l12 & 0xffff, L2 = l12 >> 16;
    if (a.memo) {
      int n1 = 0, n2 = 0;
      Compact1 c;
      CompactPrep q;
      q.x.path = -1; q.x.pos = 0; q.x.edit = 0; q.x.orient = 0; q.y = q.x;
#pragma unroll
      for (int k = 0; k < K; k++) {
        if (x.live[k]) { n1++; q.x.path = x.path[k]; q.x.pos = x.pos[k]; q.x.edit = x.ef[k] & 0xff; q.x.orient = x.ef[k] >> 8; }
        if (y.live[k]) { n2++; q.y.path = y.path[k]; q.y.pos = y.pos[k]; q.y.edit = y.ef[k] & 0xff; q.y.orient = y.ef[k] >> 8; }
      }
      int code = (a.lt_codes > 0 && l12 == a.len_combo0) ? 0 : -1;
      if (code < 0 && a.n_codes > 1) {
#pragma unroll
        for (int k = 3; k >= 1; k--) if (k < a.lt_codes && a.len_combo[k] == l12) code = k;
      }
      if (n1 == 1 && n2 == 1 && q.x.path == q.y.path && code >= 0 && q.x.orient != q.y.orient && q.x.edit < 7 && q.y.edit < 7) {
        const bool fwd = q.x.pos < q.y.pos;
        const bool ok = fwd ? (q.x.orient == 0) : (q.x.orient == 1);
        const int dist = fwd ? q.y.pos - q.x.pos + L2 : q.x.pos - q.y.pos + L1;
        if (ok && dist >= 0 && dist < a.ins_n) {
          c.lc = code; c.L1 = L1; c.L2 = L2;
          q.dist = dist; q.scores = true; q.skip = false;
          q.memo_idx = ((code * 7 + q.x.edit) * 7 + q.y.edit) * a.ins_n + dist;
          const double tfl = code == 0 ? a.tfloor0 : a.tfloor_c[code], lfl = code == 0 ? a.logfloor0 : a.logfloor_c[code];
          const double2 m = a.memo[q.memo_idx];
          if (cap) *cap = PairVal{m.x, m.y, code, 1};
          compact_cover(a, c, q, m.x);
          __builtin_nontemporal_store(m.x, &a.probs[i]);
          const bool floored = m.x < tfl;
          lsum += floored ? lfl : m.y - a.log_two_T;
          zeros += (int)floored;
          return;
        }
      }
    }
    const double acc = score_regs<K>(a, x, y, L1, L2);
    finish_read(a, i, acc, L1, L2, lsum, zeros, cap);
}

template <int K, bool GEN>
__device__ __forceinline__ void paired_regs_body(const PairedArgs& a, int lb, int slot_lo, int slot_hi, int block_lo, int block_hi,
                                                 double& lsum, int& zeros, unsigned long long* tl = nullptr, int4* wave_lds = nullptr) {
  bool first_pair = true;
#ifdef GAML_GEN_STAMPS
  const unsigned long long tb_ = wall_clock64();
#endif
  for (int i = slot_lo + (lb - block_lo) * kBlock + threadIdx.x; i < slot_hi; i += (block_hi - block_lo) * kBlock) {
    const int t = i - a.n0;
    const uint32_t l12 = a.len12[t];
    const size_t at = K == 2 ? (size_t)2 * (i - a.n0) : (size_t)2 * (a.n01 - a.n0) + (size_t)4 * (i - a.n01);
    int4 r1[K], r2[K];
#pragma unroll
    for (int k = 0; k < K; k++) { r1[k] = a.inl[0][at + k]; r2[k] = a.inl[1][at + k]; }
    if (tl && first_pair) { asm volatile("s_waitcnt vmcnt(0)" ::: "memory"); if ((threadIdx.x & 63) == 0) tl[2] = (unsigned long long)wall_clock64() + (r1[0].x == 0x12345 ? 1 : 0); }
    RegCands<K> x, y;
    const bool m1 = cands_from_records<K>(a.m[0], r1, x), m2 = cands_from_records<K>(a.m[1], r2, y);
    if (tl && first_pair) { asm volatile("s_waitcnt vmcnt(0)" ::: "memory"); if ((threadIdx.x & 63) == 0) tl[3] = (unsigned long long)wall_clock64() + (x.pos[0] == 0x12345 ? 1 : 0); }
    const bool dirty = r1[0].x == kDirtyWid;
    const bool general = !dirty && (m1 || m2);
    if (!dirty && !general) score_cands_and_finish<K>(a, i, l12, x, y, lsum, zeros);
    if (tl && first_pair) { asm volatile("s_waitcnt vmcnt(0)" ::: "memory"); if ((threadIdx.x & 63) == 0) tl[5] = (unsigned long long)wall_clock64() + (lsum == 0.12345 ? 1 : 0); }
    first_pair = false;
    if (GEN && !GAML_GEN_OFF(2) && __any(general)) {
      int4* const slot = gen_wave_slot(wave_lds, general);
#ifdef GAML_GEN_STAMPS
      const unsigned long long tc0_ = wall_clock64();
#endif
      if (general) {
        double acc;
        const int L1 = l12 & 0xffff, L2 = l12 >> 16;
        int4 priv[K == 2 ? 2 * kGenCands : 1];
        if (K == 2 && general_pair_staged<K>(a, r1, r2, L1, L2, acc, slot ? slot : priv)) finish_read(a, i, acc, L1, L2, lsum, zeros);
        else { const GenOut o = general_pair_call(kernel_args_address(), i, -1, -1, slot); lsum += o.add; zeros += o.zeros; }
      }
#ifdef GAML_GEN_STAMPS
      if (general) { asm volatile("s_waitcnt vmcnt(0) lgkmcnt(0)" ::: "memory"); const unsigned long long tc1_ = wall_clock64(); atomicAdd(&g_gen_stamp[5], tc1_ - tc0_); atomicAdd(&g_gen_stamp[6], 1ull); atomicAdd(&g_gen_stamp[21], tc0_ - tb_); }
#endif
    }
  }
}

template <bool GEN>
__device__ __forceinline__ void paired_delta_body(const PairedArgs& a, int db, int delta_blocks, double& lsum, int& zeros, int4* wave_lds = nullptr) {
  for (int dj = db * kBlock + threadIdx.x; dj < a.dstate[kDsDirty]; dj += delta_blocks * kBlock) {
    const int i = a.dirty_slots[dj];
    const int sp = a.dirty_spill[dj];
    int4 r0[4], r1[4];
#pragma unroll
    for (int k = 0; k < 2; k++) { r0[k] = a.dirty_recs[0][4 * (size_t)dj + k]; r1[k] = a.dirty_recs[1][4 * (size_t)dj + k]; }
    const uint32_t l12 = (uint32_t)r0[0].w;
    const int c0 = r1[0].w & 0xff, c1 = (r1[0].w >> 8) & 0xff;
    bool general = false;
    if (__all(sp >= 0 || (c0 <= 2 && c1 <= 2))) {
      if (sp < 0) {
        RegCands<2> x, y;
        const int4 q0[2] = {r0[0], r0[1]}, q1[2] = {r1[0], r1[1]};
        const bool m0 = cands_from_records<2>(a.m[0], q0, x), m1 = cands_from_records<2>(a.m[1], q1, y);
        general = m0 || m1;
        if (!general) score_cands_and_finish<2>(a, i, l12, x, y, lsum, zeros);
      }
    } else if (sp < 0) {
#pragma unroll
      for (int k = 2; k < 4; k++) { r0[k] = a.dirty_recs[0][4 * (size_t)dj + k]; r1[k] = a.dirty_recs[1][4 * (size_t)dj + k]; }
      RegCands<4> x, y;
      const bool m0 = cands_from_records<4>(a.m[0], r0, x), m1 = cands_from_records<4>(a.m[1], r1, y);
      general = m0 || m1;
      if (!general) score_cands_and_finish<4>(a, i, l12, x, y, lsum, zeros);
    }
    if (GEN) {
      if (!GAML_GEN_OFF(4) && __any(general)) {
        int4* const slot = gen_wave_slot(wave_lds, general);
        if (general) { const GenOut o = general_pair_call(kernel_args_address(), i, dj, -1, slot); lsum += o.add; zeros += o.zeros; }
      }
    } else if (general) {
      lsum += __builtin_nan("");
    }
  }
}

struct DeltaPatch { int dj, slot, spill, pad; int4 rec[2][4]; };
struct DeltaPatch2 { int dj, slot, spill, pad; int4 rec[2][2]; };
__device__ __forceinline__ void mark_dirty_slot(int s, unsigned long long* rec8_0, int n0, int4* inl_0, int n01, int n_main, int4* first_0) {
  if (s < n0) rec8_0[s] = ~0ull - 1;
  else {
    if (s < n01) inl_0[(size_t)2 * (s - n0)].x = -2;
    else if (s < n_main) inl_0[(size_t)2 * (n01 - n0) + (size_t)4 * (s - n01)].x = -2;
    first_0[s - n0].x = -2;
  }
}
template <class Patch, int K>
__global__ __launch_bounds__(kBlock) void apply_delta_patch_kernel(const Patch* patch, int n, int* slots, int* spill, int4* rec0, int4* rec1, int mark_from,
                                                                   unsigned long long* rec8_0, int n0, int4* inl_0, int n01, int n_main, int4* first_0) {
  for (int t = blockIdx.x * kBlock + threadIdx.x; t < n; t += gridDim.x * kBlock) {
    const Patch p = patch[t];
    slots[p.dj] = p.slot;
    spill[p.dj] = p.spill;
#pragma unroll
    for (int k = 0; k < 4; k++) {
      rec0[4 * (size_t)p.dj + k] = k < K ? p.rec[0][k < K ? k : 0] : make_int4(-1, 0, 0, 0);
      rec1[4 * (size_t)p.dj + k] = k < K ? p.rec[1][k < K ? k : 0] : make_int4(-1, 0, 0, 0);
    }
    if (mark_from >= 0 && p.dj >= mark_from) mark_dirty_slot(p.slot, rec8_0, n0, inl_0, n01, n_main, first_0);
  }
}

template <bool TICKET, bool GEN, bool TL, bool COV = false>
__device__ __forceinline__ void paired_main_body(const PairedArgs& a, int lb, double* sh_s, int* sh_z, int4* gen_lds) {
  double lsum = 0.0;
  int zeros = 0;
  unsigned long long* tl = TL ? a.timeline + ((size_t)blockIdx.x * (kBlock / 64) + (threadIdx.x >> 6)) * 8 : nullptr;
  if (TL && (threadIdx.x & 63) == 0) { tl[0] = wall_clock64(); tl[7] = lb < a.blocks0 ? 0 : (lb < a.blocks01 ? 1 : 2); }
  if (GAML_TIMING_X(8) && lb >= a.blocks0a) {
  } else if (GAML_TIMING_X(16) && lb < a.blocks0a) {
  } else if (lb < a.blocks0) {
    GAML_FRESH_ARGS(c, a)
    const bool wide = c.memo && (COV || !c.cov_bits);
    const SlotRange rg = compact_range(c, lb);
    const bool stat = wide && lb < c.blocks0a;
    if (!TL && wide && c.n_codes == 1) {
      if (stat) paired_static4_body<GEN, false, true, COV>(c, rg, lsum, zeros);
      else paired_compact4_body<GEN, false, true, COV>(c, rg, lsum, zeros);
    } else {
      __shared__ uint32_t sh_combo[256];
      __shared__ double sh_floor[256], sh_logfloor[256], sh_tfloor[256], sh_covthr[COV ? 256 : 1];
      for (int k = threadIdx.x; k < c.n_codes; k += kBlock) { sh_combo[k] = c.len_combo[k]; sh_floor[k] = c.floor_c[k]; sh_logfloor[k] = c.logfloor_c[k]; sh_tfloor[k] = c.tfloor_c ? c.tfloor_c[k] : 0.0; if (COV) sh_covthr[k] = c.covthr_c[k]; }
      __syncthreads();
      PairedArgs b = c;
      b.len_combo = sh_combo; b.floor_c = sh_floor; b.logfloor_c = sh_logfloor; b.tfloor_c = sh_tfloor;
      if (COV) b.covthr_c = sh_covthr;
      if (TL && (threadIdx.x & 63) == 0) tl[1] = wall_clock64();
      if (stat) paired_static4_body<GEN, TL, false, COV>(b, rg, lsum, zeros);
      else if (wide) paired_compact4_body<GEN, TL, false, COV>(b, rg, lsum, zeros);
      else paired_compact_body<GEN>(b, rg, lsum, zeros);
    }
  } else {
    int4* const wave_lds = GEN ? gen_lds + (threadIdx.x >> 6) * 2 * kOvfCap : nullptr;
    if (lb < a.blocks01) {
      GAML_FRESH_ARGS(c, a)
      paired_regs_body<2, GEN>(c, lb, c.n0, c.n01, c.blocks0, c.blocks01, lsum, zeros, tl, wave_lds);
    } else if (lb < a.blocks012) {
      GAML_FRESH_ARGS(c, a)
      paired_regs_body<4, GEN>(c, lb, c.n01, c.n_main, c.blocks01, c.blocks012, lsum, zeros, nullptr, wave_lds);
    } else {
      GAML_FRESH_ARGS(c, a)
      paired_delta_body<GEN>(c, lb - c.blocks012, c.main_blocks - c.blocks012, lsum, zeros, wave_lds);
    }
  }
  block_reduce(lsum, zeros, sh_s, sh_z);
  if (TL && (threadIdx.x & 63) == 0) tl[6] = wall_clock64();
  if (TICKET) {
    GAML_FRESH_ARGS(c, a)
    grid_finish(lsum, zeros, lb, c.total_blocks, c.part_sum, c.part_zero, c.ticket, c.out,
                c.cov_bits ? -1.0 : 0.0, c.n_reads, sh_s, sh_z, c.status_out, c.status_a, c.status_b);
  } else if (threadIdx.x == 0) {
    a.part_sum[lb] = lsum;
    a.part_zero[lb] = zeros;
  }
}

__global__ __launch_bounds__(kBlock) void finish_partials_kernel(const double* part_sum, const int* part_zero, int n_partials,
                                                                 double* out, double bad_bases, double n_reads,
                                                                 double* status_out = nullptr, double status_a = 0.0, double status_b = 0.0) {
  __shared__ double sh_s[kBlock / 64];
  __shared__ int sh_z[kBlock / 64];
  double ts = 0; int tz = 0;
  for (int b = threadIdx.x; b < n_partials; b += kBlock) { ts += part_sum[b]; tz += part_zero[b]; }
  block_reduce(ts, tz, sh_s, sh_z);
  if (threadIdx.x == 0) {
    out[0] = ts; out[1] = (double)tz; if (bad_bases >= 0) out[2] = bad_bases; out[3] = n_reads;
    if (status_out) { status_out[0] = status_a; status_out[1] = status_b; }
  }
}

constexpr int kOvfMaxBlocks = 1024;

template <class Src>
__device__ __forceinline__ int wave_gather(const MateView& v, const Src& src, int4* lds, int lane) {
  const int cnt = src.count();
  int total = 0;
  for (int base = 0; base < cnt; base += 64) {
    const int k = base + lane;
    int mine = 0;
    int4 r = make_int4(-1, 0, 0, 0), o = make_int4(0, 0, -1, 0);
    if (k < cnt) {
      r = src.get(k);
      if (r.x >= 0) { const Occ12 e = v.occ12[r.x]; o = occ_from_compact((unsigned long long)e.lo | ((unsigned long long)e.hi << 32), e.rank); }
      if (o.z >= 0) mine = o.w >= 0 ? 1 : v.multi_off[-o.w] - v.multi_off[-o.w - 1];
    }
    int incl = mine;
    for (int d = 1; d < 64; d <<= 1) { int t = __shfl_up(incl, d, 64); if (lane >= d) incl += t; }
    const int wave_total = __shfl(incl, 63, 64);
    const int at = total + incl - mine;
    if (total + wave_total > kOvfCap) return -1;
    if (mine == 1 && o.w >= 0) {
      lds[at] = make_int4(o.z, r.y + o.x, (r.z & 0x1ff) | ((r.y >= o.y) ? 0x200 : 0), o.w);
    } else if (mine > 0) {
      const int s = -o.w - 1;
      for (int q = 0; q < mine; q++) {
        const int4 oo = v.multi[v.multi_off[s] + q];
        lds[at + q] = make_int4(oo.z, r.y + oo.x, (r.z & 0x1ff) | ((r.y >= oo.y) ? 0x200 : 0), oo.w);
      }
    }
    total += wave_total;
  }
  return total;
}

template <class Src>
__device__ __forceinline__ double wave_score_pair(const PairedArgs& a, const Src& s1, const Src& s2, int L1, int L2, int4* c1, int4* c2, int lane) {
  const int n1 = wave_gather(a.m[0], s1, c1, lane);
  const int n2 = wave_gather(a.m[1], s2, c2, lane);
  double acc = 0.0;
  if (n1 < 0 || n2 < 0) {
    if (lane == 0) acc = paired_general_src(a, s1, s2, L1, L2);
    return acc;
  }
  __builtin_amdgcn_wave_barrier();
  for (int m = 0; m < 2; m++) {
    int4* c = m == 0 ? c1 : c2;
    const int n = m == 0 ? n1 : n2;
    for (int x = lane; x < n; x += 64) {
      int4 me = c[x];
      bool live = (me.z & 0x200) != 0;
      for (int y = 0; y < n && live; y++) {
        const int4 ot = c[y];
        if (y != x && (ot.z & 0x200) && ot.x == me.x && ot.y == me.y && (ot.w > me.w || (ot.w == me.w && y > x))) live = false;
      }
      if (live) me.z |= 0x400;
      c[x].z = me.z;
    }
  }
  __builtin_amdgcn_wave_barrier();
  const int pairs = n1 * n2;
  for (int idx = lane; idx < pairs; idx += 64) {
    const int4 xr = c1[idx / n2];
    const int4 yr = c2[idx % n2];
    if ((xr.z & 0x400) && (yr.z & 0x400) && xr.x == yr.x) {
      Cand x, y;
      x.path = xr.x; x.pos = xr.y; x.edit = xr.z & 0xff; x.orient = (xr.z >> 8) & 1;
      y.path = yr.x; y.pos = yr.y; y.edit = yr.z & 0xff; y.orient = (yr.z >> 8) & 1;
      acc += pair_term(a, x, y, L1, L2);
    }
  }
  for (int off = 32; off > 0; off >>= 1) acc += __shfl_xor(acc, off, 64);
  __builtin_amdgcn_wave_barrier();
  return acc;
}

template <bool TICKET>
__device__ __forceinline__ void paired_overflow_body(const PairedArgs& a, int ovf_block, int ovf_blocks, double* sh_s, int* sh_z,
                                                     int4 (*cand)[2][kOvfCap]) {
  const int lane = threadIdx.x & 63, wave = threadIdx.x >> 6;
  const int wave_global = ovf_block * (kBlock / 64) + wave;
  const int n_waves = ovf_blocks * (kBlock / 64);
  const int n_table = a.n - a.n_main;
  const int n_items = n_table + a.dstate[kDsSpill];
  double lsum = 0.0;
  int zeros = 0;
  int4* c1 = cand[wave][0];
  int4* c2 = cand[wave][1];
  for (int item = wave_global; item < n_items; item += n_waves) {
    if (item < n_table) {
      const int i = a.n_main + item;
      const int4 r1 = a.m[0].first[i - a.n0], r2 = a.m[1].first[i - a.n0];
      const uint32_t l12 = a.len12[i - a.n0];
      if (r1.x == kDirtyWid) continue;
      const int L1 = l12 & 0xffff, L2 = l12 >> 16;
      const double acc = wave_score_pair(a, TableSrc{&a.m[0], r1}, TableSrc{&a.m[1], r2}, L1, L2, c1, c2, lane);
      if (lane == 0) finish_read(a, i, acc, L1, L2, lsum, zeros);
    } else {
      const int sp = item - n_table;
      const int i = a.spill_slot[sp];
      const uint32_t l12 = i < a.n0 ? a.len_combo[a.len_code[i]] : a.len12[i - a.n0];
      const int L1 = l12 & 0xffff, L2 = l12 >> 16;
      const int2 g0 = a.spill_rng[0][sp], g1 = a.spill_rng[1][sp];
      const double acc = wave_score_pair(a, ListSrc{a.spill_recs[0] + g0.x, g0.y}, ListSrc{a.spill_recs[1] + g1.x, g1.y}, L1, L2, c1, c2, lane);
      if (lane == 0) finish_read(a, i, acc, L1, L2, lsum, zeros);
    }
  }
  block_reduce(lsum, zeros, sh_s, sh_z);
  if (TICKET) {
    grid_finish(lsum, zeros, a.main_blocks + ovf_block, a.total_blocks, a.part_sum, a.part_zero, a.ticket, a.out,
                a.cov_bits ? -1.0 : 0.0, a.n_reads, sh_s, sh_z, a.status_out, a.status_a, a.status_b);
  } else if (threadIdx.x == 0) {
    a.part_sum[a.main_blocks + ovf_block] = lsum;
    a.part_zero[a.main_blocks + ovf_block] = zeros;
  }
}

#ifndef GAML_GEN_WAVES
#define GAML_GEN_WAVES 4
#endif
template <bool TICKET, bool GEN = false, bool TL = false, bool COV = false>
__global__ __launch_bounds__(kBlock, GEN ? GAML_GEN_WAVES : 5) void paired_score_kernel(PairedArgs a) {
  __shared__ double sh_s[kBlock / 64];
  __shared__ int sh_z[kBlock / 64];
  __shared__ int4 cand[kBlock / 64][2][kOvfCap];
  const int lb = a.total_blocks - 1 - (int)blockIdx.x;
#if GAML_LEAN_ENTRY && defined(__HIP_DEVICE_COMPILE__)
  if (!TL && lb < a.blocks0a && a.memo && (COV || !a.cov_bits) && a.n_codes == 1) {
    double lsum = 0.0;
    int zeros = 0;
    if (!GAML_TIMING_X(16))
    paired_static4_body<GEN, false, true, COV>(a, SlotRange{0, a.n0a, lb, a.blocks0a}, lsum, zeros);
    block_reduce(lsum, zeros, sh_s, sh_z);
    if (TICKET) grid_finish(lsum, zeros, lb, a.total_blocks, a.part_sum, a.part_zero, a.ticket, a.out, COV ? -1.0 : 0.0, a.n_reads, sh_s, sh_z, a.status_out, a.status_a, a.status_b);
    else if (threadIdx.x == 0) { a.part_sum[lb] = lsum; a.part_zero[lb] = zeros; }
    return;
  }
  if (lb < a.main_blocks) paired_main_body<TICKET, GEN, TL, COV>(a, lb, sh_s, sh_z, &cand[0][0][0]);
  else if (GAML_GEN_OFF(16)) { if (threadIdx.x == 0) { a.part_sum[lb] = 0.0; a.part_zero[lb] = 0; } }
  else {
    GAML_FRESH_ARGS(c, a)
    paired_overflow_body<TICKET>(c, lb - c.main_blocks, c.total_blocks - c.main_blocks, sh_s, sh_z, cand);
  }
#else
  if (lb < a.main_blocks) paired_main_body<TICKET, GEN, TL, COV>(a, lb, sh_s, sh_z, &cand[0][0][0]);
  else paired_overflow_body<TICKET>(a, lb - a.main_blocks, a.total_blocks - a.main_blocks, sh_s, sh_z, cand);
#endif
}

constexpr int kMaxSets = 8;
struct SetDev {
  const Occ12* occ12[2];
  const int* multi_off[2];
  const int4* multi[2];
  const double* tfloor_c;
  double tfloor0;
  double two_T, log_two_T;
  double* part_sum;
  int* part_zero;
  uint32_t* cov_bits;
  const int* slot_base;
};
struct MultiSets { int n; int pad_; const unsigned char* chg[2]; SetDev set[kMaxSets]; };

constexpr int kTfCodes = 16;
template <bool COV = false>
__device__ __forceinline__ PairedArgs with_set(const PairedArgs& a, const SetDev& sd, const double* tfloor_lds = nullptr) {
  PairedArgs b = a;
  if (COV) { b.cov_bits = sd.cov_bits; b.path_base = sd.slot_base; }
#pragma unroll
  for (int mt = 0; mt < 2; mt++) { b.m[mt].occ12 = sd.occ12[mt]; b.occ12[mt] = sd.occ12[mt]; b.m[mt].multi_off = sd.multi_off[mt]; b.m[mt].multi = sd.multi[mt]; }
  b.tfloor_c = tfloor_lds ? tfloor_lds : sd.tfloor_c; b.tfloor0 = sd.tfloor0; b.two_T = sd.two_T; b.log_two_T = sd.log_two_T;
  b.part_sum = sd.part_sum; b.part_zero = sd.part_zero;
  return b;
}

struct MultiKernArgs { PairedArgs a; MultiSets ms; };
#if defined(__HIP_DEVICE_COMPILE__)
#define GAML_CALLEE_ARGS(name, set, COV)                                                                                             \
  const unsigned long long name##_u = ((unsigned long long)(unsigned)__builtin_amdgcn_readfirstlane((int)(kernargs >> 32)) << 32) |  \
                                      (unsigned)__builtin_amdgcn_readfirstlane((int)kernargs);          \
  const __attribute__((address_space(4))) MultiKernArgs* name##_p = (const __attribute__((address_space(4))) MultiKernArgs*)name##_u; \
  const PairedArgs name##_0 = name##_p->a;                                                                                           \
  const PairedArgs name = (set) >= 0 ? with_set<COV>(name##_0, name##_p->ms.set[set]) : name##_0;
#else
#define GAML_CALLEE_ARGS(name, set, COV) const PairedArgs& name = *(const PairedArgs*)nullptr;
#endif
template <bool COV>
__device__ __forceinline__ GenOut compact_general_impl(unsigned long long kernargs, int i, int set) {
  GAML_CALLEE_ARGS(a, set, COV)
  GenOut o{0.0, 0};
  compact_general(a, i, o.add, o.zeros);
  return o;
}
__device__ __noinline__ GenOut compact_general_call(unsigned long long kernargs, int i, int set) { return compact_general_impl<false>(kernargs, i, set); }
__device__ __noinline__ GenOut compact_general_call_cov(unsigned long long kernargs, int i, int set) { return compact_general_impl<true>(kernargs, i, set); }
template <bool COV>
__device__ __forceinline__ GenOut general_pair_impl(unsigned long long kernargs, int i, int dj, int set, int4* lds) {
  GAML_CALLEE_ARGS(a, set, COV)
// ... 646 lines not shown
```

### gaml_amd/csrc/occ_device.hip.h

```cpp
#pragma once

namespace {

constexpr int kOccMaxDesc = 32;

struct OccDesc { long long off; int slot, start; };
struct OccScatterArgs {
  const OccPre* pool[2];
  Occ12* dst[2];
  int* dst_list[2];
  Occ12* clr[2];
  const int* clr_list[2];
  unsigned* stamp[2];
  int* dup;
  int n_desc, total[2], n_clr[2];
  unsigned serial;
  OccDesc desc[2][kOccMaxDesc];
};

__global__ void __launch_bounds__(kBlock) occ_scatter_kernel(const OccScatterArgs a) {
  const int t0 = a.total[0], t01 = t0 + a.total[1], c0 = t01 + a.n_clr[0], n = c0 + a.n_clr[1];
  for (int i = blockIdx.x * blockDim.x + threadIdx.x; i < n; i += gridDim.x * blockDim.x) {
    if (i < t01) {
      const int mt = i < t0 ? 0 : 1;
      const int j = mt ? i - t0 : i;
      int d = 0;
      while (d + 1 < a.n_desc && a.desc[mt][d + 1].start <= j) d++;
      const OccDesc& D = a.desc[mt][d];
      const OccPre e = a.pool[mt][D.off + (j - D.start)];
      Occ12* o = a.dst[mt] + e.wid;
      o->lo = e.lo; o->hi = e.hi | ((unsigned)D.slot << 16); o->rank = e.rank;
      a.dst_list[mt][j] = e.wid;
      if (atomicExch(a.stamp[mt] + e.wid, a.serial) == a.serial) *(volatile int*)a.dup = 1;
    } else {
      const int mt = i < c0 ? 0 : 1;
      const int j = mt ? i - c0 : i - t01;
      Occ12* o = a.clr[mt] + a.clr_list[mt][j];
      o->lo = ~0u; o->hi = ~0u; o->rank = -1;
    }
  }
}

bool paired_resident_route(const gaml_hip_ctx* c, const PairedSet& s) {
  return c->host_results && c->direct_write && KNOB(c, 8) == 0 && KNOB(c, 13) == 0;
}

bool occdev_route_ok(const gaml_hip_ctx* c, PairedSet& s) {
  PairedSet::OccDev& D = s.occdev;
  if (!c->occ_route || KNOB(c, 17) != 0 || !paired_resident_route(c, s) || !s.persist.valid) return false;
  if (s.cfg.penalty_constant > 0) return false;
  if (s.planner.last_was_incremental()) return false;
  const std::vector<int32_t>& ids = s.planner.ids();
  if (ids.empty() || ids.size() > (size_t)kOccMaxDesc) return false;
  D.key.clear();
  for (int32_t id : ids) {
    const PathMemo& pm = s.planner.memo(id);
    if (!pm.pre_plain[0] || !pm.pre_plain[1]) return false;
    D.key.push_back((uint64_t)(uint32_t)id << 32 | pm.serial);
  }
  for (const auto& k : D.shared) if (k == D.key) return false;
  return true;
}

void occdev_note_shared(PairedSet::OccDev& D) {
  constexpr size_t kShared = 16;
  if (D.shared.size() < kShared) D.shared.push_back(D.key);
  else { D.shared[D.shared_next] = D.key; D.shared_next = (D.shared_next + 1) % kShared; }
}

int occdev_reserve(gaml_hip_ctx* c, PairedSet& s, size_t n_windows, size_t n_occ, hipStream_t st) {
  PairedSet::OccDev& D = s.occdev;
  if (D.cap_w > 0 && n_windows <= D.cap_w && n_occ <= D.cap_list) return 0;
  HIP_TRY(c, hipStreamSynchronize(st));
  D.cap_w = std::max(std::max<size_t>(4 * n_windows, (size_t)1 << 18), D.cap_w);
  D.cap_list = std::max(std::max<size_t>(2 * n_occ, (size_t)1 << 16), D.cap_list);
  for (int mt = 0; mt < 2; mt++) {
    for (int k = 0; k < 2; k++) {
      HIP_TRY(c, D.tab[mt][k].reserve(D.cap_w * sizeof(Occ12)));
      HIP_TRY(c, hipMemsetAsync(D.tab[mt][k].p, 0xff, D.cap_w * sizeof(Occ12), st));
      HIP_TRY(c, D.list[mt][k].reserve(D.cap_list * sizeof(int32_t)));
      D.list_n[mt][k] = 0;
    }
    HIP_TRY(c, D.stamp[mt].reserve(D.cap_w * sizeof(uint32_t)));
    HIP_TRY(c, hipMemsetAsync(D.stamp[mt].p, 0, D.cap_w * sizeof(uint32_t), st));
  }
  D.serial = 0;
  return 0;
}

int occdev_upload(gaml_hip_ctx* c, PairedSet& s, hipStream_t st, size_t* bytes) {
  PairedSet::OccDev& D = s.occdev;
  const std::vector<int32_t>& ids = s.planner.ids();
  auto missing = [&](const PathMemo& pm, int mt) { return pm.dev_off[mt] < 0 || pm.dev_gen[mt] != D.pool_gen; };
  size_t need[2] = {0, 0}, whole[2] = {0, 0};
  for (int32_t id : ids)
    for (int mt = 0; mt < 2; mt++) { const PathMemo& pm = s.planner.memo(id); whole[mt] += pm.pre[mt].size(); if (missing(pm, mt)) need[mt] += pm.pre[mt].size(); }
  if (D.pool_used[0] + need[0] > D.pool_cap[0] || D.pool_used[1] + need[1] > D.pool_cap[1]) {
    HIP_TRY(c, hipStreamSynchronize(st));
    for (int mt = 0; mt < 2; mt++) {
      if (2 * whole[mt] > D.pool_cap[mt]) {
        D.pool_cap[mt] = std::max<size_t>(8 * whole[mt], 2 * D.pool_cap[mt]);
        HIP_TRY(c, D.pool[mt].reserve(D.pool_cap[mt] * sizeof(OccPre)));
      }
      D.pool_used[mt] = 0;
      need[mt] = whole[mt];
    }
    D.pool_gen++;
    D.compactions++;
  }
  *bytes = (need[0] + need[1]) * sizeof(OccPre);
  if (need[0] + need[1] == 0) return 0;
  HIP_TRY(c, D.stage.reserve(*bytes));
  OccPre* sp = (OccPre*)D.stage.p;
  for (int mt = 0; mt < 2; mt++) {
    const size_t at = D.pool_used[mt];
    size_t k = 0;
    for (int32_t id : ids) {
      PathMemo& pm = s.planner.memo(id);
      if (!missing(pm, mt)) continue;
      pm.dev_off[mt] = (int64_t)(at + k);
      pm.dev_gen[mt] = D.pool_gen;
      if (!pm.pre[mt].empty()) memcpy(sp + k, pm.pre[mt].data(), pm.pre[mt].size() * sizeof(OccPre));
      k += pm.pre[mt].size();
    }
    if (k) HIP_TRY(c, hipMemcpyAsync(D.pool[mt].as<OccPre>() + at, sp, k * sizeof(OccPre), hipMemcpyHostToDevice, st));
    D.pool_used[mt] = at + k;
    sp += k;
  }
  return 0;
}

int occdev_launch(gaml_hip_ctx* c, PairedSet& s, hipStream_t st, size_t* bytes) {
  PairedSet::OccDev& D = s.occdev;
  const std::vector<int32_t>& ids = s.planner.ids();
  if (D.pool_cap[0] == 0 || D.pool_cap[1] == 0) {
    for (int mt = 0; mt < 2; mt++) {
      size_t all = 0;
      for (int32_t id : ids) all += s.planner.memo(id).pre[mt].size();
      D.pool_cap[mt] = std::max<size_t>(16 * all, (size_t)1 << 10);
      HIP_TRY(c, D.pool[mt].reserve(D.pool_cap[mt] * sizeof(OccPre)));
      D.pool_used[mt] = 0;
    }
    D.pool_gen++;
  }
  size_t n_occ[2] = {0, 0};
  for (int32_t id : ids) for (int mt = 0; mt < 2; mt++) n_occ[mt] += s.planner.memo(id).pre[mt].size();
  const size_t n_windows = std::max(s.mate[0].wins.size(), s.mate[1].wins.size());
  if (int e = occdev_reserve(c, s, n_windows, std::max(n_occ[0], n_occ[1]), st)) return e;
  if (int e = occdev_upload(c, s, st, bytes)) return e;
  HIP_TRY(c, D.dup.reserve(sizeof(int)));
  *(volatile int*)D.dup.p = 0;
  if (++D.serial == 0) {
    for (int mt = 0; mt < 2; mt++) HIP_TRY(c, hipMemsetAsync(D.stamp[mt].p, 0, D.cap_w * sizeof(uint32_t), st));
    D.serial = 1;
  }
  const int cur = (int)(D.serial & 1), other = cur ^ 1;
  OccScatterArgs a;
  memset(&a, 0, sizeof(a));
  a.n_desc = (int)ids.size();
  for (int mt = 0; mt < 2; mt++) {
    a.pool[mt] = D.pool[mt].as<OccPre>();
    a.dst[mt] = D.tab[mt][cur].as<Occ12>();
    a.dst_list[mt] = D.list[mt][cur].as<int>();
    a.clr[mt] = D.tab[mt][other].as<Occ12>();
    a.clr_list[mt] = D.list[mt][other].as<int>();
    a.stamp[mt] = D.stamp[mt].as<unsigned>();
    int start = 0;
    for (size_t k = 0; k < ids.size(); k++) {
      const PathMemo& pm = s.planner.memo(ids[k]);
      a.desc[mt][k] = OccDesc{(long long)pm.dev_off[mt], (int)k, start};
      start += (int)pm.pre[mt].size();
    }
    a.total[mt] = start;
    a.n_clr[mt] = D.list_n[mt][other];
    D.list_n[mt][cur] = start;
    D.list_n[mt][other] = 0;
  }
  a.dup = (int*)D.dup.dev;
  a.serial = D.serial;
  const int items = a.total[0] + a.total[1] + a.n_clr[0] + a.n_clr[1];
  if (items > 0) {
    hipLaunchKernelGGL(occ_scatter_kernel, dim3((unsigned)std::min(512, (items + kBlock - 1) / kBlock)), dim3(kBlock), 0, st, a);
    HIP_TRY(c, hipGetLastError());
  }
  return 0;
}

const Occ12* occdev_table(const PairedSet& s, int mt) { return s.occdev.tab[mt][s.occdev.serial & 1].as<Occ12>(); }

void paired_images_refresh(PairedSet& s) {
  if (!s.occdev.image_stale) return;
  s.planner.rebuild_images(s.mate, s.image);
  s.occdev.image_stale = false;
}

}
```

### gaml_amd/csrc/paired_launch.hip.h

```cpp
#pragma once

namespace {

int paired_host_tabs(gaml_hip_ctx* c, PairedSet& s) {
  if (!s.ins_tab.empty() || !s.floor_tab.empty()) return 0;
  const double c0 = s.cfg.min_prob_start, k0 = s.cfg.min_prob_per_base;
  auto ins = [&](int d) {
    double z = ((double)d - s.cfg.insert_mean) / s.cfg.insert_std;
    return std::exp(-z * z / 2.0) / (std::sqrt(2 * M_PI) * s.cfg.insert_std);
  };
  const int kInsCap = 1 << 22;
  s.ins_tab.clear();
  for (int d = 0; d < kInsCap; d++) {
    double v = ins(d);
    if (v == 0.0 && (double)d > s.cfg.insert_mean) break;
    s.ins_tab.push_back(v);
  }
  if ((int)s.ins_tab.size() >= kInsCap)
    return fail(c, GAML_HIP_EINVAL, "insert_std too large: the insert-size table would exceed 4M entries");
  int smax = s.mate[0].max_len + s.mate[1].max_len;
  s.floor_tab.resize(smax + 1);
  s.logfloor_tab.resize(smax + 1);
  for (int v = 0; v <= smax; v++) {
    s.floor_tab[v] = std::exp(c0 + k0 * v);
// ... 13 lines not shown
  double* d = s.tabs.as<double>();
  size_t at = 0;
  auto up = [&](const std::vector<double>& v) -> hipError_t {
    hipError_t e = v.empty() ? hipSuccess : hipMemcpy(d + at, v.data(), v.size() * sizeof(double), hipMemcpyHostToDevice);
    at += v.size();
    return e;
  };
  HIP_TRY(c, up(s.ins_tab));
  HIP_TRY(c, up(s.floor_tab));
  HIP_TRY(c, up(s.logfloor_tab));
  HIP_TRY(c, up(s.covthr_tab));
  const int64_t n = s.mate[0].n_local();
  HIP_TRY(c, s.probs.reserve(std::max<size_t>(1, n) * sizeof(double)));
  HIP_TRY(c, s.red.init());
  HIP_TRY(c, s.bad.reserve(sizeof(unsigned long long)));
  s.tabs_uploaded = true;
  return 0;
}

int prepare_paired_structure(gaml_hip_ctx* c, PairedSet& s, const int32_t* flat, const int64_t* offs, int32_t n_paths) {
  const bool incremental = KNOB(c, 12) == 0;
  std::string err;
  if (!s.planner.begin(c->g, s.mate, flat, offs, n_paths, incremental, &err)) return fail(c, GAML_HIP_EINVAL, err);
  return 0;
}

void paired_cov_build(PairedSet& s, bool cov, PairedPrep& p) {
  p.path_base.assign(1, 0);
  p.start_off.assign(1, 0);
  p.starts.clear();
  p.slot_base.assign(1, 0);
  if (!cov) return;
  const PlanView& v = s.planner.view();
  const std::vector<int32_t>& slots = s.planner.slots();
  p.path_base.reserve(v.paths.size() + 1);
  p.start_off.reserve(v.paths.size() + 1);
  p.slot_base.assign((size_t)std::max(1, s.planner.slot_count()), 0);
  for (size_t k = 0; k < v.paths.size(); k++) {
    const PathMemo* pm = v.paths[k];
    p.starts.insert(p.starts.end(), pm->starts.begin(), pm->starts.end());
    p.start_off.push_back((int32_t)p.starts.size());
    int32_t bits = ((pm->length + 64 + 31) / 32) * 32;
    p.slot_base[(size_t)slots[k]] = p.path_base.back();
    p.path_base.push_back(p.path_base.back() + bits);
  }
}

int prepare_paired_tables_host(gaml_hip_ctx* c, PairedSet& s, PairedPrep& p, hipStream_t st = nullptr, bool device_route = false) {
  static const bool trace = getenv("GAML_HIP_TRACE_HOST") != nullptr;
  const double q0 = now_us();
  s.planner.finish(s.mate);
  PairedSet::OccDev& D = s.occdev;
  D.taken = device_route && occdev_route_ok(c, s);
  size_t up_bytes = 0;
  if (D.taken) { if (int e = occdev_launch(c, s, st, &up_bytes)) return e; }
  c->prof[6] = (double)up_bytes;
  const double q1 = now_us();
  const bool cov = s.cfg.penalty_constant > 0;
  paired_cov_build(s, cov, p);
  p.total_bits = p.path_base.back();
  p.n_paths = s.planner.n_paths();
  const double q2 = now_us();
  s.planner.apply(s.mate, s.image, !D.taken, D.image_stale);
  D.image_stale = D.taken;
  if (D.taken) D.dev_calls++; else D.host_calls++;
  p.assembled_records = s.planner.assembled(0) + s.planner.assembled(1);
  p.general = !D.taken && (!s.image[0].general_wids.empty() || !s.image[1].general_wids.empty());
  if (trace) fprintf(stderr, "pass2: finish %.1f us, starts %.1f us, images %.1f us\n", q1 - q0, q2 - q1, now_us() - q2);
  return 0;
}

}
#include "paired_tables.hip.h"
namespace {

double tfloor_for(double floor, double two_T) {
  if (!(floor > 0.0)) return 0.0;
  double x = floor * two_T;
  for (int k = 0; k < 64 && x > 0.0 && (std::nextafter(x, 0.0) / two_T) >= floor; k++) x = std::nextafter(x, 0.0);
  for (int k = 0; k < 64 && (x / two_T) < floor; k++) x = std::nextafter(x, std::numeric_limits<double>::infinity());
  return x;
}

struct PairedLayout { size_t tfloor_off; OccLayout l0, l1; size_t sb_off, pb_off, so_off, st_off, total; };

void paired_cov_layout(const PairedPrep& p, size_t at, PairedLayout& L) {
  L.sb_off = align16(at);
  L.pb_off = align16(L.sb_off + p.slot_base.size() * sizeof(int32_t));
  L.so_off = align16(L.pb_off + p.path_base.size() * sizeof(int32_t));
  L.st_off = align16(L.so_off + p.start_off.size() * sizeof(int32_t));
  L.total = align16(L.st_off + p.starts.size() * sizeof(int32_t));
}
void paired_cov_pack(const PairedPrep& p, const PairedLayout& L, char* dst) {
  memcpy(dst + L.sb_off, p.slot_base.data(), p.slot_base.size() * sizeof(int32_t));
  memcpy(dst + L.pb_off, p.path_base.data(), p.path_base.size() * sizeof(int32_t));
  memcpy(dst + L.so_off, p.start_off.data(), p.start_off.size() * sizeof(int32_t));
  if (!p.starts.empty()) memcpy(dst + L.st_off, p.starts.data(), p.starts.size() * sizeof(int32_t));
}
size_t paired_cov_ints(const PairedPrep& p) {
  return p.slot_base.size() + p.path_base.size() + p.start_off.size() + p.starts.size() + 16;
}

PairedLayout paired_layout(const PairedSet& s, const PairedPrep& p, const size_t* pad_to = nullptr) {
  PairedLayout L;
  L.tfloor_off = 0;
  const size_t hdr = align16(256 * sizeof(double));
  L.l0 = layout_image(s.image[0], hdr, pad_to ? pad_to[0] : 0);
  L.l1 = layout_image(s.image[1], L.l0.end, pad_to ? pad_to[1] : 0);
  L.sb_off = L.pb_off = L.l1.end; L.so_off = L.st_off = 0; L.total = L.l1.end;
  if (s.cfg.penalty_constant > 0) paired_cov_layout(p, L.l1.end, L);
  return L;
}

void paired_pack_thresholds(const PairedSet& s, const PairedLayout& L, double two_T, char* dst) {
  double tf[256];
  const size_t nc = std::min<size_t>(256, s.pt.len_combo.size());
  for (size_t ci = 0; ci < nc; ci++) {
    const int L0 = (int)(s.pt.len_combo[ci] & 0xffff), L1 = (int)(s.pt.len_combo[ci] >> 16);
// ... 229 lines not shown

CovArgs paired_cov_args(const PairedSet& s, const PairedPrep& p, const PairedLayout& L, const char* arena) {
  CovArgs ca;
  ca.bits = s.cov_bits.as<uint32_t>();
  ca.path_base = (const int*)(arena + L.pb_off);
  ca.start_off = (const int*)(arena + L.so_off);
  ca.starts = (const int*)(arena + L.st_off);
  ca.n_paths = p.n_paths;
  ca.total_words = p.total_bits / 32;
  ca.cov_move = s.cfg.step;
  ca.far = s.cfg.insert_mean + 5 * s.cfg.insert_std;
  ca.bad = s.bad.as<unsigned long long>();
  return ca;
}

int paired_host_partials(gaml_hip_ctx* c, PairedSet& s, int first_set, int n_sets, int n_partials, double** d_sum, int** d_zero) {
  const size_t per = (size_t)(4 * kMaxBlocks + kOvfMaxBlocks);
  HIP_TRY(c, s.h_part_sum.reserve(per * sizeof(double) * kMaxSets));
  HIP_TRY(c, s.h_part_zero.reserve(per * sizeof(int) * kMaxSets));
  *d_sum = (double*)s.h_part_sum.dev;
  *d_zero = (int*)s.h_part_zero.dev;
  double* hs = (double*)s.h_part_sum.p;
  int* hz = (int*)s.h_part_zero.p;
  for (int k = first_set; k < first_set + n_sets; k++) {
    for (int b2 = 0; b2 < n_partials; b2++) { hs[(size_t)k * per + b2] = std::numeric_limits<double>::quiet_NaN(); hz[(size_t)k * per + b2] = INT_MIN; }
    s.last_blocks[k] = n_partials;
  }
  s.host_part_stride = per;
  return 0;
}

int launch_paired(gaml_hip_ctx* c, PairedSet& s, PairedPrep& p, int32_t total_len, hipStream_t st, double* out4) {
  const double tpp = now_us();
  if (int e = prepare_paired_tables(c, s)) return e;
  const double tp0 = now_us();
  if (int e = prepare_paired_tables_host(c, s, p, st, true)) return e;
  const double t_after_host = now_us();
  c->prof[1] = t_after_host - tp0;
  gpu_probe(st, c->warm_buf.p, "before table sync");
  if (int e = paired_sync_tables(c, s, st)) return e;
  const double tp1 = now_us();
  c->prof[4] = tp1 - t_after_host;
  if (tp1 - t_after_host > 1000.0 && getenv("GAML_HIP_TRACE_HOST")) fprintf(stderr, "table sync took %.0f us (evaluation %lld of the set, rebuild active %d slice %d)\n", tp1 - t_after_host, (long long)s.eval_count, (int)s.rebuild.active, s.rebuild.next_slice);

  const bool cov = s.cfg.penalty_constant > 0;
  const int tl = total_len == 0 ? 1 : total_len;
  const bool resident = paired_resident_route(c, s);
  PairedLayout L;
  memset(&L, 0, sizeof(L));
  int slot = -1;
  const char* arena = nullptr;
  SetDev sd;
  s.occdev.check_dup = s.occdev.taken;
  if (s.occdev.taken) {
    PairedLayout Lt;
    Lt.tfloor_off = s.persist.off_tfloor;
    paired_pack_thresholds(s, Lt, (double)(2 * tl), (char*)s.persist.dev);
    _mm_sfence();
    paired_persist_view(s, total_len, sd);
    for (int mt = 0; mt < 2; mt++) sd.occ12[mt] = occdev_table(s, mt);
    c->prof[6] += 256.0 * sizeof(double);
  } else if (resident) {
    if (int e = paired_persist_update(c, s, (double)(2 * tl), st, &p, cov ? &L : nullptr)) return e;
    paired_persist_view(s, total_len, sd);
    c->prof[6] = (double)s.persist.last_bytes;
    if (cov) arena = (const char*)s.persist.dev;
  } else {
    L = paired_layout(s, p);
    char* wp = nullptr;
    if (int e = arena_acquire(c, s.arena, L.total, st, &slot, &wp)) return e;
    paired_pack(s, p, L, wp);
    paired_pack_thresholds(s, L, (double)(2 * tl), wp);
    if (int e = arena_commit(c, s.arena, slot, L.total, st)) return e;
    arena = (const char*)s.arena.dev[slot];
    paired_set_view(s, L, arena, total_len, sd);
    c->prof[6] = (double)L.total;
  }
  const double tp2 = now_us();
  c->prof[3] = tp2 - tp1;

  PairedArgs a;
  GridPlan gp;
  paired_base_args(c, s, a, gp);
  const int64_t n = s.mate[0].n_local();
  if (cov) {
    size_t words = (size_t)p.total_bits / 32;
    if (words * 4 > s.cov_bits.cap) { HIP_TRY(c, hipStreamSynchronize(st)); HIP_TRY(c, s.cov_bits.reserve(std::max<size_t>(4, words * 4))); }
    HIP_TRY(c, hipMemsetAsync(s.cov_bits.p, 0, std::max<size_t>(4, words * 4), st));
    HIP_TRY(c, hipMemsetAsync(s.bad.p, 0, sizeof(unsigned long long), st));
    a.cov_bits = s.cov_bits.as<uint32_t>();
    a.path_base = (const int*)(arena + L.sb_off);
  }
  const bool gen_set = a.n_main > 0 && p.general;
  const int n_partials = gp.total_blocks;
  sd.part_sum = s.red.part_sum.as<double>();
  sd.part_zero = s.red.part_zero.as<int>();
  if (c->host_results && n > 0) { if (int e = paired_host_partials(c, s, 0, 1, n_partials, &sd.part_sum, &sd.part_zero)) return e; }
  s.last_blocks[0] = n > 0 ? n_partials : 0;
  s.last_host_partials = c->host_results;
  s.last_sets = 1;
  paired_apply_set(a, sd);
  a.out = out4;
  a.timeline = nullptr;
  const bool timeline = KNOB(c, 3) == 8;
  if (timeline) {
    HIP_TRY(c, s.h_timeline.reserve((size_t)(4 * kMaxBlocks + kOvfMaxBlocks + 256) * (kBlock / 64) * 8 * sizeof(unsigned long long)));
    memset(s.h_timeline.p, 0, s.h_timeline.cap);
    a.timeline = (unsigned long long*)s.h_timeline.dev;
    s.timeline_waves = a.total_blocks * (kBlock / 64);
  }

  std::pair<hipEvent_t, hipEvent_t>* ev = nullptr;
  if (n > 0) {
    if (c->event_timing && (c->event_tick++ % c->event_every) == 0) { if (int e = take_events(c, &ev)) return e; }
    int fin_mode = c->host_results ? 2 : (KNOB(c, 2) ? KNOB(c, 2) - 1 : 1);
    double* status_out = nullptr;
    if (fin_mode != 2 && c->status_dst && !c->status_done) { status_out = c->status_dst; c->status_done = true; }
    if (fin_mode == 0) { a.status_out = status_out; a.status_a = c->status_a; a.status_b = c->status_b; }
    s.last_total_blocks = n_partials;
    const dim3 grid(a.total_blocks), block(kBlock);
    hipEvent_t e0 = ev ? ev->first : nullptr, e1 = ev ? ev->second : nullptr;
#define GAML_LAUNCH_SCORE(...) hipExtLaunchKernelGGL((paired_score_kernel<__VA_ARGS__>), grid, block, KNOB(c, 1), st, e0, e1, 0, a)
#ifdef GAML_HIP_DEV
    if (timeline) GAML_LAUNCH_SCORE(false, false, true);
    else
#endif
    if (gen_set) { if (fin_mode) GAML_LAUNCH_SCORE(false, true); else GAML_LAUNCH_SCORE(true, true); }
    else if (cov && a.memo && KNOB(c, 21) == 0) { if (fin_mode) GAML_LAUNCH_SCORE(false, false, false, true); else GAML_LAUNCH_SCORE(true, false, false, true); }
    else if (fin_mode) GAML_LAUNCH_SCORE(false, false);
    else GAML_LAUNCH_SCORE(true, false);
#undef GAML_LAUNCH_SCORE
    HIP_TRY(c, hipGetLastError());
    if (fin_mode == 1) {
      hipLaunchKernelGGL(finish_partials_kernel, dim3(1), dim3(kBlock), 0, st, a.part_sum, a.part_zero, n_partials, out4, cov ? -1.0 : 0.0, (double)n, status_out, c->status_a, c->status_b);
      HIP_TRY(c, hipGetLastError());
    }
  } else {
    s.last_total_blocks = 0;
    if (!c->host_results) HIP_TRY(c, hipMemsetAsync(out4, 0, 4 * sizeof(double), st));
  }
  if (cov && c->defer_cov) {
    int idx = 0;
    for (size_t i = 0; i < c->paireds.size(); i++) if (c->paireds[i].get() == &s) idx = (int)i;
    c->pending_cov.push_back(gaml_hip_ctx::PendingCov{idx, paired_cov_args(s, p, L, arena), out4});
  } else if (cov && n > 0 && p.total_bits > 0) {
    const CovArgs ca = paired_cov_args(s, p, L, arena);
    hipLaunchKernelGGL(coverage_sweep_kernel, dim3(grid_for(ca.total_words)), dim3(kBlock), 0, st, ca);
    HIP_TRY(c, hipGetLastError());
  }
  if (cov && n > 0 && !c->defer_cov) {
    hipLaunchKernelGGL(store_bad_bases_kernel, dim3(1), dim3(64), 0, st, s.bad.as<unsigned long long>(), out4, 1.0);
    HIP_TRY(c, hipGetLastError());
  }
  if (slot >= 0) { if (int e = arena_release(c, s.arena, slot, st)) return e; }
  c->prof[5] = now_us() - tp2;
  if (now_us() - tpp > 5000.0 && getenv("GAML_HIP_TRACE_HOST"))
    fprintf(stderr, "launch_paired: fixed tables %.2f ms, pass 2 %.2f, table sync %.2f, per-call tables %.2f, launches %.2f\n", (tp0 - tpp) * 1e-3, (t_after_host - tp0) * 1e-3,
            (tp1 - t_after_host) * 1e-3, (tp2 - tp1) * 1e-3, (now_us() - tp2) * 1e-3);
  if (!c->event_timing || ev) {
    c->stat_algo_bytes += 16.0 * (double)p.assembled_records + 16.0 * (double)n;
    c->stat_launches++;
  }
  c->t_host_us += t_after_host;
  return 0;
}

bool paired_multi_capable(const gaml_hip_ctx* c, const PairedSet& s) {
  if (KNOB(c, 3) != 0 || KNOB(c, 4) != 0 || !s.floor_positive) return false;
  return !(s.cfg.penalty_constant > 0) || KNOB(c, 21) == 0;
}

int launch_paired_multi(gaml_hip_ctx* c, PairedSet& s, int first, int n_sets, const PairedLayout* L, const PairedPrep* preps, const int32_t* total_lens,
                        const char* arena, size_t stride, hipStream_t st, const unsigned char* const* chg = nullptr) {
  PairedArgs a;
  GridPlan gp;
  paired_base_args(c, s, a, gp);
  if (!a.memo) return fail(c, GAML_HIP_ESTATE, "multi-set launch without a memo (caller must check paired_multi_capable)");
  const int64_t n = s.mate[0].n_local();
  bool any_set = false;
  for (int k = first; k < first + n_sets; k++) any_set = any_set || (a.n_main > 0 && preps[k].general);
// ... 91 lines not shown
```

### include/gaml_hip_debug.h

```cpp
#ifndef GAML_HIP_DEBUG_H_
#define GAML_HIP_DEBUG_H_

#include "gaml_hip.h"

#ifdef __cplusplus
extern "C" {
#endif

int gaml_hip_debug_sam_logprob(gaml_hip_ctx* ctx, const char* target, int32_t target_len, const char* read, int32_t read_len,
                               const char* sam_line, int64_t sam_len, double mismatch_prob, double* logprob_out,
                               int32_t* band_lo, int32_t* band_hi, int32_t band_cap);
int gaml_hip_debug_sam_shape(const char* sam_line, int64_t len, int32_t total_len, int32_t* out6, uint32_t* ops, int32_t cap);
int32_t gaml_hip_debug_sam_band(const char* sam_line, int64_t len, int32_t total_len, int32_t* fields10, int32_t* row0,
                                int32_t* lo, int32_t* hi, int32_t cap);

int gaml_hip_debug_prepare(gaml_hip_ctx* ctx, const int32_t* paths, const int64_t* path_offs, int32_t n_paths);
int64_t gaml_hip_debug_occurrences(gaml_hip_ctx* ctx, int readset, int mate, int32_t* out5, int64_t cap);
int64_t gaml_hip_debug_table_occurrences(gaml_hip_ctx* ctx, int readset, int mate, int32_t* out5, int64_t cap, int64_t* info3);
int32_t gaml_hip_debug_cov_layout(gaml_hip_ctx* ctx, int readset, int32_t* slot_base, int32_t cap_slots, int32_t* path_base, int32_t* start_off,
                                  int32_t* slots, int32_t cap_paths, int32_t* starts, int32_t cap_starts, int32_t* counts4);
int32_t gaml_hip_debug_window_walk(gaml_hip_ctx* ctx, int readset, int mate, int32_t window_id, int32_t* out, int32_t cap);
int gaml_hip_debug_timeline(gaml_hip_ctx* ctx, int rs, unsigned long long* out, int64_t cap_waves);

int gaml_hip_debug_set_knob(gaml_hip_ctx* ctx, int knob, int value);
int gaml_hip_debug_fold_check(gaml_hip_ctx* ctx, int readset, int64_t* out6);
int gaml_hip_debug_radix_sort(gaml_hip_ctx* ctx, uint64_t* keys, uint64_t* vals, int64_t n, int begin_bit, int end_bit, uint64_t* run_max);
int gaml_hip_debug_static_check(gaml_hip_ctx* ctx, int readset, int64_t* out8);
int gaml_hip_debug_tables_check(gaml_hip_ctx* ctx, int readset, int64_t* out8);
int32_t gaml_hip_debug_block_partials(gaml_hip_ctx* ctx, int readset, int32_t set, double* sums, int32_t* zeros, int32_t cap, int32_t* layout8);

int gaml_hip_debug_occ_route(gaml_hip_ctx* ctx, int readset, int64_t* out6);
int gaml_hip_debug_occ_check(gaml_hip_ctx* ctx, int readset, int64_t* out4);

int32_t gaml_hip_debug_batch_bad_bases(gaml_hip_ctx* ctx, int readset, int64_t* out, int32_t cap);

#ifdef __cplusplus
}
#endif
#endif
```

Before: 66.07 billion reads/s.

## Add dense per-path occurrence tables cached on device across path sets

New measurement: 72.26 billion reads/s, median of 6. 1.09x the previous value.

```diff
diff --git a/gaml_amd/api.py b/gaml_amd/api.py
--- a/gaml_amd/api.py
+++ b/gaml_amd/api.py
@@ -199,6 +199,8 @@
         L.gaml_hip_debug_set_knob.argtypes = [vp, C.c_int, C.c_int]
     if hasattr(L, "gaml_hip_debug_occ_route"):
         L.gaml_hip_debug_occ_route.argtypes = [vp, C.c_int, _i64p]
+    if hasattr(L, "gaml_hip_debug_occ_dense"):
+        L.gaml_hip_debug_occ_dense.argtypes = [vp, C.c_int, _i64p]
     if hasattr(L, "gaml_hip_debug_occ_check"):
         L.gaml_hip_debug_occ_check.argtypes = [vp, C.c_int, _i64p]
     if hasattr(L, "gaml_hip_debug_batch_bad_bases"):
@@ -780,6 +782,12 @@
         return {"device": int(out[0]), "host": int(out[1]), "fallbacks": int(out[2]), "compactions": int(out[3]),
                 "pool_entries": int(out[4]), "shared_combinations": int(out[5])}
 
+    def debug_occ_dense(self, rs):
+        out = np.zeros(8, np.int64)
+        self._check(_lib.gaml_hip_debug_occ_dense(self._h, rs, out))
+        return {"dense": int(out[0]), "scatter": int(out[1]), "built": int(out[2]), "restarts": int(out[3]),
+                "arena_entries": int(out[4]), "arena_capacity": int(out[5]), "table_entries": int(out[6]), "windows": int(out[7])}
+
     def debug_occ_check(self, rs):
         out = np.zeros(4, np.int64)
         rc = _lib.gaml_hip_debug_occ_check(self._h, rs, out)
diff --git a/gaml_amd/csrc/ctx.hip.h b/gaml_amd/csrc/ctx.hip.h
--- a/gaml_amd/csrc/ctx.hip.h
+++ b/gaml_amd/csrc/ctx.hip.h
@@ -305,6 +305,13 @@
     int32_t list_n[2][2] = {{0, 0}, {0, 0}};
     uint32_t serial = 0;
     PinBuf dup;
+    DevBuf dtab[2];
+    size_t dense_cap[2] = {0, 0}, dense_used[2] = {0, 0}, dense_n[2] = {0, 0};
+    uint32_t dense_gen = 0;
+    DenseMate dense_view[2] = {};
+    bool dense = false;
+    bool last_dense = false;
+    int64_t dense_calls = 0, dense_built = 0, dense_restarts = 0;
     bool taken = false;
     bool check_dup = false;
     bool image_stale = false;
@@ -314,7 +321,7 @@
     int64_t dev_calls = 0, host_calls = 0, fallbacks = 0, compactions = 0;
     void release() {
       for (int mt = 0; mt < 2; mt++) {
-        pool[mt].release(); stamp[mt].release();
+        pool[mt].release(); stamp[mt].release(); dtab[mt].release();
         for (int k = 0; k < 2; k++) { tab[mt][k].release(); list[mt][k].release(); }
       }
       stage.release(); dup.release();
@@ -429,7 +436,7 @@
   double aln_us = 0;
   double aln_stage_us[5] = {0, 0, 0, 0, 0};
   int64_t aln_batches = 0;
-  int knobs[24] = {0};
+  int knobs[32] = {0};
   bool direct_write = false;
   int32_t peers = 1;
   std::string err;
diff --git a/gaml_amd/csrc/debug_api.hip.h b/gaml_amd/csrc/debug_api.hip.h
--- a/gaml_amd/csrc/debug_api.hip.h
+++ b/gaml_amd/csrc/debug_api.hip.h
@@ -104,7 +104,7 @@
 }
 
 int gaml_hip_debug_set_knob(gaml_hip_ctx* c, int knob, int value) {
-  if (!c || knob < 0 || knob >= 24) return GAML_HIP_EINVAL;
+  if (!c || knob < 0 || knob >= 32) return GAML_HIP_EINVAL;
   if (c->multi) { for (int k = 0; k < gaml::multi_num_shards(c->multi); k++) gaml::multi_shard(c->multi, k)->knobs[knob] = value; return GAML_HIP_OK; }
   c->knobs[knob] = value;
   return GAML_HIP_OK;
@@ -333,6 +333,19 @@
   return GAML_HIP_OK;
 }
 
+int gaml_hip_debug_occ_dense(gaml_hip_ctx* c, int rs, int64_t* out8) {
+  MULTI_SHARD0(c);
+  int64_t* out6 = out8;
+  if (!c || !out6 || rs < 0 || rs >= (int)c->handles.size() || c->handles[rs].kind != 1) return fail(c, GAML_HIP_EINVAL, "bad arguments");
+  const PairedSet& ps = *c->paireds[c->handles[rs].idx];
+  const PairedSet::OccDev& D = ps.occdev;
+  out8[6] = D.last_dense ? (int64_t)D.dense_view[0].n : 0;
+  out8[7] = (int64_t)ps.mate[0].wins.size();
+  out6[0] = D.dense_calls; out6[1] = D.dev_calls - D.dense_calls; out6[2] = D.dense_built; out6[3] = D.dense_restarts;
+  out6[4] = (int64_t)(D.dense_used[0] + D.dense_used[1]); out6[5] = (int64_t)(D.dense_cap[0] + D.dense_cap[1]);
+  return GAML_HIP_OK;
+}
+
 int gaml_hip_debug_occ_check(gaml_hip_ctx* c, int rs, int64_t* out4) {
   MULTI_SHARD0(c);
   if (!c || !out4 || rs < 0 || rs >= (int)c->handles.size() || c->handles[rs].kind != 1) return fail(c, GAML_HIP_EINVAL, "bad arguments");
@@ -348,6 +361,20 @@
     im.build(ps.mate[mt].wins.size(), v, mt);
     const size_t n = im.occ12.size();
     std::vector<Occ12> dev(n);
+    if (D.last_dense) {
+      const DenseMate& dv = D.dense_view[mt];
+      std::vector<Occ12> ta(dv.n), tb(dv.n);
+      if (dv.n) HIP_TRY(c, hipMemcpy(ta.data(), dv.A, dv.n * sizeof(Occ12), hipMemcpyDeviceToHost));
+      if (dv.n) HIP_TRY(c, hipMemcpy(tb.data(), dv.B, dv.n * sizeof(Occ12), hipMemcpyDeviceToHost));
+      for (size_t w = 0; w < n; w++) {
+        const Occ12 none{~0u, ~0u, -1};
+        const Occ12 ea = w < ta.size() ? ta[w] : none, eb = w < tb.size() ? tb[w] : none;
+        dev[w] = ea.hi != ~0u ? ea : Occ12{eb.lo, eb.hi | 0x10000u, eb.rank};
+        if (ea.hi != ~0u && eb.hi != ~0u) out4[2]++;
+      }
+      for (size_t w = n; w < ta.size(); w++)
+        if (ta[w].hi != ~0u || tb[w].hi != ~0u) out4[2]++;
+    } else
     if (n) HIP_TRY(c, hipMemcpy(dev.data(), occdev_table(ps, mt), n * sizeof(Occ12), hipMemcpyDeviceToHost));
     for (size_t w = 0; w < n; w++) {
       const Occ12& h = im.occ12[w];
diff --git a/gaml_amd/csrc/host_model.cc b/gaml_amd/csrc/host_model.cc
--- a/gaml_amd/csrc/host_model.cc
+++ b/gaml_amd/csrc/host_model.cc
@@ -971,6 +971,7 @@
       occ_prepack(pm.occ[mt], pm.pre[mt]);
       pm.pre_plain[mt] = occ_pre_plain(pm.pre[mt]);
       pm.dev_off[mt] = -1;
+      pm.tab_off[mt] = -1;
       pm.occ_valid[mt] = true;
     }
   };
diff --git a/gaml_amd/csrc/host_model.h b/gaml_amd/csrc/host_model.h
--- a/gaml_amd/csrc/host_model.h
+++ b/gaml_amd/csrc/host_model.h
@@ -233,6 +233,8 @@
   bool pre_plain[2] = {false, false};
   int64_t dev_off[2] = {-1, -1};
   uint32_t dev_gen[2] = {0, 0};
+  int64_t tab_off[2] = {-1, -1};
+  uint32_t tab_gen[2] = {0, 0};
   int64_t assembled[2] = {0, 0};
   std::vector<int32_t> starts;
   int32_t length = 0;
diff --git a/gaml_amd/csrc/kernels.hip.h b/gaml_amd/csrc/kernels.hip.h
--- a/gaml_amd/csrc/kernels.hip.h
+++ b/gaml_amd/csrc/kernels.hip.h
@@ -20,6 +20,8 @@
   const double* mism_pow;
   const double* match_pow;
 };
+
+struct DenseMate { const Occ12* A; const Occ12* B; unsigned n, pad_; };
 
 struct PairedArgs {
   int total_blocks, blocks0a, n0a, n_codes;
@@ -74,7 +76,31 @@
   double n_reads;
   double* status_out;
   double status_a, status_b;
+  DenseMate dense[2];
+  int* dup;
 };
+
+template <bool RANK>
+__device__ __forceinline__ Occ12 dense_lookup(const DenseMate& d, unsigned w, bool& both) {
+  const unsigned off = min(w, d.n) * 12u;
+  const Occ12* pa = (const Occ12*)((const char*)d.A + off);
+  const Occ12* pb = (const Occ12*)((const char*)d.B + off);
+  Occ12 ea, eb;
+  ea.lo = pa->lo; ea.hi = pa->hi; ea.rank = RANK ? pa->rank : -1;
+  eb.lo = pb->lo; eb.hi = pb->hi; eb.rank = RANK ? pb->rank : -1;
+  const bool in_a = ea.hi != ~0u, in_b = eb.hi != ~0u;
+  both |= in_a & in_b;
+  Occ12 e;
+  e.lo = in_a ? ea.lo : eb.lo; e.hi = in_a ? ea.hi : (eb.hi | 0x10000u); e.rank = in_a ? ea.rank : eb.rank;
+  return e;
+}
+__device__ __forceinline__ unsigned long long dense_occ8(const PairedArgs& a, int mt, unsigned w, bool& both) {
+  const Occ12 e = dense_lookup<false>(a.dense[mt], w, both);
+  return (unsigned long long)e.lo | ((unsigned long long)e.hi << 32);
+}
+__device__ __forceinline__ void dense_raise(int* dup, bool both) {
+  if (both) { *(volatile int*)dup = 1; __threadfence_system(); }
+}
 
 struct Cand { int path, pos, edit, orient, rank, k; bool valid; };
 
@@ -288,13 +314,13 @@
   bool valid[K], live[K];
 };
 
-template <int K>
-__device__ __forceinline__ bool cands_from_records(const MateView& v, const int4 (&r)[K], RegCands<K>& c) {
+template <int K, bool D = false>
+__device__ __forceinline__ bool cands_from_records(const MateView& v, const int4 (&r)[K], RegCands<K>& c, const DenseMate dm = DenseMate{}, bool* both = nullptr) {
   int4 o[K];
   bool multi = false;
   Occ12 e[K];
 #pragma unroll
-  for (int k = 0; k < K; k++) e[k] = v.occ12[r[k].x >= 0 ? r[k].x : 0];
+  for (int k = 0; k < K; k++) e[k] = D ? dense_lookup<true>(dm, (unsigned)r[k].x, *both) : v.occ12[r[k].x >= 0 ? r[k].x : 0];
 #pragma unroll
   for (int k = 0; k < K; k++) o[k] = occ_from_compact((unsigned long long)e[k].lo | ((unsigned long long)e[k].hi << 32), e[k].rank);
 #pragma unroll
@@ -545,11 +571,12 @@
   return lb < a.blocks0a ? SlotRange{0, a.n0a, lb, a.blocks0a} : SlotRange{a.n0a, a.n0, lb - a.blocks0a, a.blocks0 - a.blocks0a};
 }
 
-template <bool GEN>
+template <bool GEN, bool D = false>
 __device__ __forceinline__ void paired_compact_body(const PairedArgs& a, const SlotRange rg, double& lsum, int& zeros) {
   const int stride = rg.blocks * kBlock, hi = rg.hi;
   int i0 = rg.lo + rg.lb * kBlock + threadIdx.x;
   if (i0 >= hi) return;
+  bool shared = false;
   Compact1 c0, c1;
   compact_load(a, i0, true, c0);
   compact_load(a, i0 + stride, i0 + stride < hi, c1);
@@ -566,10 +593,10 @@
     const bool d0 = c0.r1 == kDirty8, d1 = c1.r1 == kDirty8;
     if (d0) { c0.r1 = kNone8; c0.r2 = kNone8; }
     if (d1) { c1.r1 = kNone8; c1.r2 = kNone8; }
-    c0.o1 = c0.r1 != kNone8 ? occ8_of(a.occ12[0], (unsigned)(c0.r1 & 0xffffff)) : kNone8;
-    c0.o2 = c0.r2 != kNone8 ? occ8_of(a.occ12[1], (unsigned)(c0.r2 & 0xffffff)) : kNone8;
-    c1.o1 = c1.r1 != kNone8 ? occ8_of(a.occ12[0], (unsigned)(c1.r1 & 0xffffff)) : kNone8;
-    c1.o2 = c1.r2 != kNone8 ? occ8_of(a.occ12[1], (unsigned)(c1.r2 & 0xffffff)) : kNone8;
+    c0.o1 = D ? dense_occ8(a, 0, c0.r1 != kNone8 ? (unsigned)(c0.r1 & 0xffffff) : ~0u, shared) : (c0.r1 != kNone8 ? occ8_of(a.occ12[0], (unsigned)(c0.r1 & 0xffffff)) : kNone8);
+    c0.o2 = D ? dense_occ8(a, 1, c0.r2 != kNone8 ? (unsigned)(c0.r2 & 0xffffff) : ~0u, shared) : (c0.r2 != kNone8 ? occ8_of(a.occ12[1], (unsigned)(c0.r2 & 0xffffff)) : kNone8);
+    c1.o1 = D ? dense_occ8(a, 0, c1.r1 != kNone8 ? (unsigned)(c1.r1 & 0xffffff) : ~0u, shared) : (c1.r1 != kNone8 ? occ8_of(a.occ12[0], (unsigned)(c1.r1 & 0xffffff)) : kNone8);
+    c1.o2 = D ? dense_occ8(a, 1, c1.r2 != kNone8 ? (unsigned)(c1.r2 & 0xffffff) : ~0u, shared) : (c1.r2 != kNone8 ? occ8_of(a.occ12[1], (unsigned)(c1.r2 & 0xffffff)) : kNone8);
     CompactPrep q0, q1;
     compact_prep(a, c0, q0);
     compact_prep(a, c1, q1);
@@ -583,6 +610,7 @@
     c0 = n0v; c1 = n1v;
     i0 = j0;
   }
+  if (D) dense_raise(a.dup, shared);
 }
 
 constexpr int kPairZero = -1, kPairOther = -(1 << 20);
@@ -623,7 +651,7 @@
   return state;
 }
 
-template <bool GEN, bool TL = false, bool ONE = false, bool COV = false>
+template <bool GEN, bool TL = false, bool ONE = false, bool COV = false, bool D = false>
 __device__ __forceinline__ void paired_compact4_body(const PairedArgs& a, const SlotRange rg, double& lsum, int& zeros) {
   const unsigned stride = (unsigned)rg.blocks * kBlock, n0 = (unsigned)rg.hi;
   unsigned long long* tl = TL ? a.timeline + ((size_t)blockIdx.x * (kBlock / 64) + (threadIdx.x >> 6)) * 8 : nullptr;
@@ -634,6 +662,7 @@
   const char* const occ1 = (const char*)a.occ12[1];
   const char* const memo = (const char*)a.memo;
   char* const probs = (char*)a.probs;
+  bool shared = false;
   const uint32_t l12_one = ONE ? a.len_combo[0] : 0u;
   const double logfloor_one = ONE ? a.logfloor_c[0] : 0.0, tfloor_one = ONE ? a.tfloor_c[0] : 0.0, log2T = a.log_two_T;
   const double covthr_one = COV && ONE ? a.covthr0 : 0.0;
@@ -648,6 +677,12 @@
     GAML_STAMP(2, r1[0].x ^ r1[1].x ^ r1[2].x ^ r1[3].x ^ r2[0].x ^ r2[3].x)
 #pragma unroll
     for (int k = 0; k < 4; k++) {
+      if (D) {
+        const Occ12 d1 = dense_lookup<false>(a.dense[0], r1[k].y != ~0u ? (r1[k].x & 0xffffffu) : ~0u, shared);
+        const Occ12 d2 = dense_lookup<false>(a.dense[1], r2[k].y != ~0u ? (r2[k].x & 0xffffffu) : ~0u, shared);
+        o1[k] = make_uint2(d1.lo, d1.hi); o2[k] = make_uint2(d2.lo, d2.hi);
+        continue;
+      }
       const Occ12* e1 = (const Occ12*)(occ0 + (r1[k].y != ~0u ? (r1[k].x & 0xffffffu) : 0u) * 12u);
       const Occ12* e2 = (const Occ12*)(occ1 + (r2[k].y != ~0u ? (r2[k].x & 0xffffffu) : 0u) * 12u);
       o1[k] = make_uint2(e1->lo, e1->hi); o2[k] = make_uint2(e2->lo, e2->hi);
@@ -695,8 +730,8 @@
         const int i = (int)(base + k * stride);
         Compact1 d;
         compact_load(a, i, true, d);
-        d.o1 = d.r1 != kNone8 ? occ8_of(a.occ12[0], (unsigned)(d.r1 & 0xffffff)) : kNone8;
-        d.o2 = d.r2 != kNone8 ? occ8_of(a.occ12[1], (unsigned)(d.r2 & 0xffffff)) : kNone8;
+        d.o1 = D ? dense_occ8(a, 0, d.r1 != kNone8 ? (unsigned)(d.r1 & 0xffffff) : ~0u, shared) : (d.r1 != kNone8 ? occ8_of(a.occ12[0], (unsigned)(d.r1 & 0xffffff)) : kNone8);
+        d.o2 = D ? dense_occ8(a, 1, d.r2 != kNone8 ? (unsigned)(d.r2 & 0xffffff) : ~0u, shared) : (d.r2 != kNone8 ? occ8_of(a.occ12[1], (unsigned)(d.r2 & 0xffffff)) : kNone8);
         const uint32_t l = a.len_combo[d.lc];
         d.L1 = l & 0xffff; d.L2 = l >> 16;
         CompactPrep q;
@@ -710,6 +745,7 @@
         if ((skip_bits >> k) & 1u) { const GenOut o = compact_general_call(kernel_args_address(), (int)(base + k * stride), -1); lsum += o.add; zeros += o.zeros; }
     }
   }
+  if (D) dense_raise(a.dup, shared);
 #undef GAML_STAMP
 }
 
@@ -743,7 +779,7 @@
   }
 }
 
-template <bool GEN, bool TL = false, bool ONE = false, bool COV = false>
+template <bool GEN, bool TL = false, bool ONE = false, bool COV = false, bool D = false>
 __device__ __forceinline__ void paired_static4_body(const PairedArgs& a, const SlotRange rg, double& lsum, int& zeros) {
   constexpr int P = GAML_STATIC_P;
   const unsigned stride = (unsigned)rg.blocks * kBlock, n0 = (unsigned)rg.hi;
@@ -759,6 +795,7 @@
   const double covthr_one = COV && ONE ? a.covthr0 : 0.0;
   unsigned base = (unsigned)rg.lo + (unsigned)rg.lb * kBlock + threadIdx.x;
   if (base >= n0) return;
+  bool shared = false;
   uint2 r1[P], r2[P];
   double2 m[P];
   unsigned lc[P];
@@ -774,6 +811,12 @@
     uint2 o1[P], o2[P];
 #pragma unroll
     for (int k = 0; k < P; k++) {
+      if (D) {
+        const Occ12 d1 = dense_lookup<false>(a.dense[0], (r1[k].x & 0xffffffu) | (0u - (unsigned)(r1[k].y == ~0u)), shared);
+        const Occ12 d2 = dense_lookup<false>(a.dense[1], (r2[k].x & 0xffffffu) | (0u - (unsigned)(r2[k].y == ~0u)), shared);
+        o1[k] = make_uint2(d1.lo, d1.hi); o2[k] = make_uint2(d2.lo, d2.hi);
+        continue;
+      }
       const unsigned w1 = (r1[k].x & 0xffffffu) & (0u - (unsigned)(r1[k].y != ~0u)), w2 = (r2[k].x & 0xffffffu) & (0u - (unsigned)(r2[k].y != ~0u));
       const Occ12* e1 = (const Occ12*)(occ0 + w1 * 12u);
       const Occ12* e2 = (const Occ12*)(occ1 + w2 * 12u);
@@ -847,6 +890,7 @@
       }
     }
   }
+  if (D) dense_raise(a.dup, shared);
 #undef GAML_STAMP
 }
 
@@ -1003,10 +1047,11 @@
     finish_read(a, i, acc, L1, L2, lsum, zeros, cap);
 }
 
-template <int K, bool GEN>
+template <int K, bool GEN, bool D = false>
 __device__ __forceinline__ void paired_regs_body(const PairedArgs& a, int lb, int slot_lo, int slot_hi, int block_lo, int block_hi,
                                                  double& lsum, int& zeros, unsigned long long* tl = nullptr, int4* wave_lds = nullptr) {
   bool first_pair = true;
+  bool shared = false;
 #ifdef GAML_GEN_STAMPS
   const unsigned long long tb_ = wall_clock64();
 #endif
@@ -1019,7 +1064,7 @@
     for (int k = 0; k < K; k++) { r1[k] = a.inl[0][at + k]; r2[k] = a.inl[1][at + k]; }
     if (tl && first_pair) { asm volatile("s_waitcnt vmcnt(0)" ::: "memory"); if ((threadIdx.x & 63) == 0) tl[2] = (unsigned long long)wall_clock64() + (r1[0].x == 0x12345 ? 1 : 0); }
     RegCands<K> x, y;
-    const bool m1 = cands_from_records<K>(a.m[0], r1, x), m2 = cands_from_records<K>(a.m[1], r2, y);
+    const bool m1 = cands_from_records<K, D>(a.m[0], r1, x, a.dense[0], &shared), m2 = cands_from_records<K, D>(a.m[1], r2, y, a.dense[1], &shared);
     if (tl && first_pair) { asm volatile("s_waitcnt vmcnt(0)" ::: "memory"); if ((threadIdx.x & 63) == 0) tl[3] = (unsigned long long)wall_clock64() + (x.pos[0] == 0x12345 ? 1 : 0); }
     const bool dirty = r1[0].x == kDirtyWid;
     const bool general = !dirty && (m1 || m2);
@@ -1043,10 +1088,12 @@
 #endif
     }
   }
-}
-
-template <bool GEN>
+  if (D) dense_raise(a.dup, shared);
+}
+
+template <bool GEN, bool D = false>
 __device__ __forceinline__ void paired_delta_body(const PairedArgs& a, int db, int delta_blocks, double& lsum, int& zeros, int4* wave_lds = nullptr) {
+  bool shared = false;
   for (int dj = db * kBlock + threadIdx.x; dj < a.dstate[kDsDirty]; dj += delta_blocks * kBlock) {
     const int i = a.dirty_slots[dj];
     const int sp = a.dirty_spill[dj];
@@ -1060,7 +1107,7 @@
       if (sp < 0) {
         RegCands<2> x, y;
         const int4 q0[2] = {r0[0], r0[1]}, q1[2] = {r1[0], r1[1]};
-        const bool m0 = cands_from_records<2>(a.m[0], q0, x), m1 = cands_from_records<2>(a.m[1], q1, y);
+        const bool m0 = cands_from_records<2, D>(a.m[0], q0, x, a.dense[0], &shared), m1 = cands_from_records<2, D>(a.m[1], q1, y, a.dense[1], &shared);
         general = m0 || m1;
         if (!general) score_cands_and_finish<2>(a, i, l12, x, y, lsum, zeros);
       }
@@ -1068,7 +1115,7 @@
 #pragma unroll
       for (int k = 2; k < 4; k++) { r0[k] = a.dirty_recs[0][4 * (size_t)dj + k]; r1[k] = a.dirty_recs[1][4 * (size_t)dj + k]; }
       RegCands<4> x, y;
-      const bool m0 = cands_from_records<4>(a.m[0], r0, x), m1 = cands_from_records<4>(a.m[1], r1, y);
+      const bool m0 = cands_from_records<4, D>(a.m[0], r0, x, a.dense[0], &shared), m1 = cands_from_records<4, D>(a.m[1], r1, y, a.dense[1], &shared);
       general = m0 || m1;
       if (!general) score_cands_and_finish<4>(a, i, l12, x, y, lsum, zeros);
     }
@@ -1081,6 +1128,7 @@
       lsum += __builtin_nan("");
     }
   }
+  if (D) dense_raise(a.dup, shared);
 }
 
 struct DeltaPatch { int dj, slot, spill, pad; int4 rec[2][4]; };
@@ -1109,7 +1157,7 @@
   }
 }
 
-template <bool TICKET, bool GEN, bool TL, bool COV = false>
+template <bool TICKET, bool GEN, bool TL, bool COV = false, bool D = false>
 __device__ __forceinline__ void paired_main_body(const PairedArgs& a, int lb, double* sh_s, int* sh_z, int4* gen_lds) {
   double lsum = 0.0;
   int zeros = 0;
@@ -1123,8 +1171,8 @@
     const SlotRange rg = compact_range(c, lb);
     const bool stat = wide && lb < c.blocks0a;
     if (!TL && wide && c.n_codes == 1) {
-      if (stat) paired_static4_body<GEN, false, true, COV>(c, rg, lsum, zeros);
-      else paired_compact4_body<GEN, false, true, COV>(c, rg, lsum, zeros);
+      if (stat) paired_static4_body<GEN, false, true, COV, D>(c, rg, lsum, zeros);
+      else paired_compact4_body<GEN, false, true, COV, D>(c, rg, lsum, zeros);
     } else {
       __shared__ uint32_t sh_combo[256];
       __shared__ double sh_floor[256], sh_logfloor[256], sh_tfloor[256], sh_covthr[COV ? 256 : 1];
@@ -1134,21 +1182,21 @@
       b.len_combo = sh_combo; b.floor_c = sh_floor; b.logfloor_c = sh_logfloor; b.tfloor_c = sh_tfloor;
       if (COV) b.covthr_c = sh_covthr;
       if (TL && (threadIdx.x & 63) == 0) tl[1] = wall_clock64();
-      if (stat) paired_static4_body<GEN, TL, false, COV>(b, rg, lsum, zeros);
-      else if (wide) paired_compact4_body<GEN, TL, false, COV>(b, rg, lsum, zeros);
-      else paired_compact_body<GEN>(b, rg, lsum, zeros);
+      if (stat) paired_static4_body<GEN, TL, false, COV, D>(b, rg, lsum, zeros);
+      else if (wide) paired_compact4_body<GEN, TL, false, COV, D>(b, rg, lsum, zeros);
+      else paired_compact_body<GEN, D>(b, rg, lsum, zeros);
     }
   } else {
     int4* const wave_lds = GEN ? gen_lds + (threadIdx.x >> 6) * 2 * kOvfCap : nullptr;
     if (lb < a.blocks01) {
       GAML_FRESH_ARGS(c, a)
-      paired_regs_body<2, GEN>(c, lb, c.n0, c.n01, c.blocks0, c.blocks01, lsum, zeros, tl, wave_lds);
+      paired_regs_body<2, GEN, D>(c, lb, c.n0, c.n01, c.blocks0, c.blocks01, lsum, zeros, tl, wave_lds);
     } else if (lb < a.blocks012) {
       GAML_FRESH_ARGS(c, a)
-      paired_regs_body<4, GEN>(c, lb, c.n01, c.n_main, c.blocks01, c.blocks012, lsum, zeros, nullptr, wave_lds);
+      paired_regs_body<4, GEN, D>(c, lb, c.n01, c.n_main, c.blocks01, c.blocks012, lsum, zeros, nullptr, wave_lds);
     } else {
       GAML_FRESH_ARGS(c, a)
-      paired_delta_body<GEN>(c, lb - c.blocks012, c.main_blocks - c.blocks012, lsum, zeros, wave_lds);
+      paired_delta_body<GEN, D>(c, lb - c.blocks012, c.main_blocks - c.blocks012, lsum, zeros, wave_lds);
     }
   }
   block_reduce(lsum, zeros, sh_s, sh_z);
@@ -1179,8 +1227,8 @@
 
 constexpr int kOvfMaxBlocks = 1024;
 
-template <class Src>
-__device__ __forceinline__ int wave_gather(const MateView& v, const Src& src, int4* lds, int lane) {
+template <bool D = false, class Src>
+__device__ __forceinline__ int wave_gather(const MateView& v, const Src& src, int4* lds, int lane, const DenseMate dm = DenseMate{}, bool* both = nullptr) {
   const int cnt = src.count();
   int total = 0;
   for (int base = 0; base < cnt; base += 64) {
@@ -1189,7 +1237,7 @@
     int4 r = make_int4(-1, 0, 0, 0), o = make_int4(0, 0, -1, 0);
     if (k < cnt) {
       r = src.get(k);
-      if (r.x >= 0) { const Occ12 e = v.occ12[r.x]; o = occ_from_compact((unsigned long long)e.lo | ((unsigned long long)e.hi << 32), e.rank); }
+      if (r.x >= 0) { const Occ12 e = D ? dense_lookup<true>(dm, (unsigned)r.x, *both) : v.occ12[r.x]; o = occ_from_compact((unsigned long long)e.lo | ((unsigned long long)e.hi << 32), e.rank); }
       if (o.z >= 0) mine = o.w >= 0 ? 1 : v.multi_off[-o.w] - v.multi_off[-o.w - 1];
     }
     int incl = mine;
@@ -1211,12 +1259,13 @@
   return total;
 }
 
-template <class Src>
-__device__ __forceinline__ double wave_score_pair(const PairedArgs& a, const Src& s1, const Src& s2, int L1, int L2, int4* c1, int4* c2, int lane) {
-  const int n1 = wave_gather(a.m[0], s1, c1, lane);
-  const int n2 = wave_gather(a.m[1], s2, c2, lane);
+template <bool D = false, class Src>
+__device__ __forceinline__ double wave_score_pair(const PairedArgs& a, const Src& s1, const Src& s2, int L1, int L2, int4* c1, int4* c2, int lane, bool* both = nullptr) {
+  const int n1 = wave_gather<D>(a.m[0], s1, c1, lane, a.dense[0], both);
+  const int n2 = wave_gather<D>(a.m[1], s2, c2, lane, a.dense[1], both);
   double acc = 0.0;
   if (n1 < 0 || n2 < 0) {
+    if (D) { *both = true; return acc; }
     if (lane == 0) acc = paired_general_src(a, s1, s2, L1, L2);
     return acc;
   }
@@ -1252,7 +1301,7 @@
   return acc;
 }
 
-template <bool TICKET>
+template <bool TICKET, bool D = false>
 __device__ __forceinline__ void paired_overflow_body(const PairedArgs& a, int ovf_block, int ovf_blocks, double* sh_s, int* sh_z,
                                                      int4 (*cand)[2][kOvfCap]) {
   const int lane = threadIdx.x & 63, wave = threadIdx.x >> 6;
@@ -1262,6 +1311,7 @@
   const int n_items = n_table + a.dstate[kDsSpill];
   double lsum = 0.0;
   int zeros = 0;
+  bool shared = false;
   int4* c1 = cand[wave][0];
   int4* c2 = cand[wave][1];
   for (int item = wave_global; item < n_items; item += n_waves) {
@@ -1271,7 +1321,7 @@
       const uint32_t l12 = a.len12[i - a.n0];
       if (r1.x == kDirtyWid) continue;
       const int L1 = l12 & 0xffff, L2 = l12 >> 16;
-      const double acc = wave_score_pair(a, TableSrc{&a.m[0], r1}, TableSrc{&a.m[1], r2}, L1, L2, c1, c2, lane);
+      const double acc = wave_score_pair<D>(a, TableSrc{&a.m[0], r1}, TableSrc{&a.m[1], r2}, L1, L2, c1, c2, lane, &shared);
       if (lane == 0) finish_read(a, i, acc, L1, L2, lsum, zeros);
     } else {
       const int sp = item - n_table;
@@ -1279,10 +1329,11 @@
       const uint32_t l12 = i < a.n0 ? a.len_combo[a.len_code[i]] : a.len12[i - a.n0];
       const int L1 = l12 & 0xffff, L2 = l12 >> 16;
       const int2 g0 = a.spill_rng[0][sp], g1 = a.spill_rng[1][sp];
-      const double acc = wave_score_pair(a, ListSrc{a.spill_recs[0] + g0.x, g0.y}, ListSrc{a.spill_recs[1] + g1.x, g1.y}, L1, L2, c1, c2, lane);
+      const double acc = wave_score_pair<D>(a, ListSrc{a.spill_recs[0] + g0.x, g0.y}, ListSrc{a.spill_recs[1] + g1.x, g1.y}, L1, L2, c1, c2, lane, &shared);
       if (lane == 0) finish_read(a, i, acc, L1, L2, lsum, zeros);
     }
   }
+  if (D) dense_raise(a.dup, shared);
   block_reduce(lsum, zeros, sh_s, sh_z);
   if (TICKET) {
     grid_finish(lsum, zeros, a.main_blocks + ovf_block, a.total_blocks, a.part_sum, a.part_zero, a.ticket, a.out,
@@ -1296,7 +1347,7 @@
 #ifndef GAML_GEN_WAVES
 #define GAML_GEN_WAVES 4
 #endif
-template <bool TICKET, bool GEN = false, bool TL = false, bool COV = false>
+template <bool TICKET, bool GEN = false, bool TL = false, bool COV = false, bool DENSE = false>
 __global__ __launch_bounds__(kBlock, GEN ? GAML_GEN_WAVES : 5) void paired_score_kernel(PairedArgs a) {
   __shared__ double sh_s[kBlock / 64];
   __shared__ int sh_z[kBlock / 64];
@@ -1307,21 +1358,21 @@
     double lsum = 0.0;
     int zeros = 0;
     if (!GAML_TIMING_X(16))
-    paired_static4_body<GEN, false, true, COV>(a, SlotRange{0, a.n0a, lb, a.blocks0a}, lsum, zeros);
+    paired_static4_body<GEN, false, true, COV, DENSE>(a, SlotRange{0, a.n0a, lb, a.blocks0a}, lsum, zeros);
     block_reduce(lsum, zeros, sh_s, sh_z);
     if (TICKET) grid_finish(lsum, zeros, lb, a.total_blocks, a.part_sum, a.part_zero, a.ticket, a.out, COV ? -1.0 : 0.0, a.n_reads, sh_s, sh_z, a.status_out, a.status_a, a.status_b);
     else if (threadIdx.x == 0) { a.part_sum[lb] = lsum; a.part_zero[lb] = zeros; }
     return;
   }
-  if (lb < a.main_blocks) paired_main_body<TICKET, GEN, TL, COV>(a, lb, sh_s, sh_z, &cand[0][0][0]);
+  if (lb < a.main_blocks) paired_main_body<TICKET, GEN, TL, COV, DENSE>(a, lb, sh_s, sh_z, &cand[0][0][0]);
   else if (GAML_GEN_OFF(16)) { if (threadIdx.x == 0) { a.part_sum[lb] = 0.0; a.part_zero[lb] = 0; } }
   else {
     GAML_FRESH_ARGS(c, a)
-    paired_overflow_body<TICKET>(c, lb - c.main_blocks, c.total_blocks - c.main_blocks, sh_s, sh_z, cand);
+    paired_overflow_body<TICKET, DENSE>(c, lb - c.main_blocks, c.total_blocks - c.main_blocks, sh_s, sh_z, cand);
   }
 #else
-  if (lb < a.main_blocks) paired_main_body<TICKET, GEN, TL, COV>(a, lb, sh_s, sh_z, &cand[0][0][0]);
-  else paired_overflow_body<TICKET>(a, lb - a.main_blocks, a.total_blocks - a.main_blocks, sh_s, sh_z, cand);
+  if (lb < a.main_blocks) paired_main_body<TICKET, GEN, TL, COV, DENSE>(a, lb, sh_s, sh_z, &cand[0][0][0]);
+  else paired_overflow_body<TICKET, DENSE>(a, lb - a.main_blocks, a.total_blocks - a.main_blocks, sh_s, sh_z, cand);
 #endif
 }
 
diff --git a/gaml_amd/csrc/occ_device.hip.h b/gaml_amd/csrc/occ_device.hip.h
--- a/gaml_amd/csrc/occ_device.hip.h
+++ b/gaml_amd/csrc/occ_device.hip.h
@@ -62,6 +62,31 @@
   return true;
 }
 
+int occdev_pool_init(gaml_hip_ctx* c, PairedSet& s) {
+  PairedSet::OccDev& D = s.occdev;
+  if (D.pool_cap[0] != 0 && D.pool_cap[1] != 0) return 0;
+  const std::vector<int32_t>& ids = s.planner.ids();
+  for (int mt = 0; mt < 2; mt++) {
+    size_t all = 0;
+    for (int32_t id : ids) all += s.planner.memo(id).pre[mt].size();
+    D.pool_cap[mt] = std::max<size_t>(16 * all, (size_t)1 << 10);
+    HIP_TRY(c, D.pool[mt].reserve(D.pool_cap[mt] * sizeof(OccPre)));
+    D.pool_used[mt] = 0;
+  }
+  D.pool_gen++;
+  return 0;
+}
+
+bool occdense_route_ok(const gaml_hip_ctx* c, PairedSet& s) {
+  const std::vector<int32_t>& ids = s.planner.ids();
+  if (ids.size() > 2 || KNOB(c, 23) != 0 || KNOB(c, 3) != 0) return false;
+  for (int32_t id : ids) {
+    const PathMemo& pm = s.planner.memo(id);
+    if (pm.pre[0].empty() || pm.pre[1].empty()) return false;
+  }
+  return true;
+}
+
 void occdev_note_shared(PairedSet::OccDev& D) {
   constexpr size_t kShared = 16;
   if (D.shared.size() < kShared) D.shared.push_back(D.key);
@@ -133,16 +158,7 @@
 int occdev_launch(gaml_hip_ctx* c, PairedSet& s, hipStream_t st, size_t* bytes) {
   PairedSet::OccDev& D = s.occdev;
   const std::vector<int32_t>& ids = s.planner.ids();
-  if (D.pool_cap[0] == 0 || D.pool_cap[1] == 0) {
-    for (int mt = 0; mt < 2; mt++) {
-      size_t all = 0;
-      for (int32_t id : ids) all += s.planner.memo(id).pre[mt].size();
-      D.pool_cap[mt] = std::max<size_t>(16 * all, (size_t)1 << 10);
-      HIP_TRY(c, D.pool[mt].reserve(D.pool_cap[mt] * sizeof(OccPre)));
-      D.pool_used[mt] = 0;
-    }
-    D.pool_gen++;
-  }
+  if (int e = occdev_pool_init(c, s)) return e;
   size_t n_occ[2] = {0, 0};
   for (int32_t id : ids) for (int mt = 0; mt < 2; mt++) n_occ[mt] += s.planner.memo(id).pre[mt].size();
   const size_t n_windows = std::max(s.mate[0].wins.size(), s.mate[1].wins.size());
@@ -186,6 +202,91 @@
   return 0;
 }
 
+constexpr int kDenseBuilds = 4;
+struct OccDenseBuildArgs { const OccPre* src[kDenseBuilds]; Occ12* dst[kDenseBuilds]; int n[kDenseBuilds]; unsigned n_tab[kDenseBuilds]; };
+
+__global__ void __launch_bounds__(kBlock) occ_dense_build_kernel(const OccDenseBuildArgs a) {
+  const int t = blockIdx.y;
+  for (int i = blockIdx.x * blockDim.x + threadIdx.x; i < a.n[t]; i += gridDim.x * blockDim.x) {
+    const OccPre e = a.src[t][i];
+    if ((unsigned)e.wid >= a.n_tab[t]) continue;
+    Occ12* o = a.dst[t] + e.wid;
+    o->lo = e.lo; o->hi = e.hi; o->rank = e.rank;
+  }
+}
+
+int occdense_prepare(gaml_hip_ctx* c, PairedSet& s, hipStream_t st, size_t* bytes) {
+  PairedSet::OccDev& D = s.occdev;
+  const std::vector<int32_t>& ids = s.planner.ids();
+  HIP_TRY(c, D.dup.reserve(sizeof(int)));
+  *(volatile int*)D.dup.p = 0;
+  auto missing = [&](const PathMemo& pm, int mt) { return pm.tab_off[mt] < 0 || pm.tab_gen[mt] != D.dense_gen; };
+  bool any = false;
+  for (int32_t id : ids) for (int mt = 0; mt < 2; mt++) any = any || missing(s.planner.memo(id), mt);
+  if (any) {
+    if (int e = occdev_pool_init(c, s)) return e;
+    if (int e = occdev_upload(c, s, st, bytes)) return e;
+    size_t top[2] = {0, 0}, tabs[2] = {0, 0};
+    for (int32_t id : ids)
+      for (int mt = 0; mt < 2; mt++) {
+        const PathMemo& pm = s.planner.memo(id);
+        if (!missing(pm, mt)) continue;
+        tabs[mt]++;
+        for (const OccPre& e : pm.pre[mt]) top[mt] = std::max(top[mt], (size_t)e.wid + 1);
+      }
+    bool restart = D.dense_cap[0] == 0;
+    for (int mt = 0; mt < 2; mt++) restart = restart || top[mt] > D.dense_n[mt] || D.dense_used[mt] + tabs[mt] * (D.dense_n[mt] + 1) > D.dense_cap[mt];
+    if (restart) {
+      HIP_TRY(c, hipStreamSynchronize(st));
+      D.dense_gen++;
+      for (int mt = 0; mt < 2; mt++) {
+        const size_t w = std::max(top[mt], s.mate[mt].wins.size());
+        D.dense_n[mt] = w + w / 4 + 8;
+        const size_t per = D.dense_n[mt] + 1, set_needs = (1 + ids.size()) * per;
+        const size_t want = KNOB(c, 24) > 0 ? (size_t)KNOB(c, 24) : std::max<size_t>(48 * per, (size_t)1 << 16);
+        D.dense_cap[mt] = std::max(want, set_needs);
+        HIP_TRY(c, D.dtab[mt].reserve(D.dense_cap[mt] * sizeof(Occ12)));
+        HIP_TRY(c, hipMemsetAsync(D.dtab[mt].p, 0xff, per * sizeof(Occ12), st));
+        D.dense_used[mt] = per;
+      }
+      if (D.dense_built > 0) D.dense_restarts++;
+    }
+    OccDenseBuildArgs a;
+    memset(&a, 0, sizeof(a));
+    int nb = 0, most = 0;
+    for (int mt = 0; mt < 2; mt++) {
+      const size_t from = D.dense_used[mt], per = D.dense_n[mt] + 1;
+      for (int32_t id : ids) {
+        PathMemo& pm = s.planner.memo(id);
+        if (!missing(pm, mt)) continue;
+        pm.tab_off[mt] = (int64_t)D.dense_used[mt];
+        pm.tab_gen[mt] = D.dense_gen;
+        D.dense_used[mt] += per;
+        a.src[nb] = D.pool[mt].as<OccPre>() + pm.dev_off[mt];
+        a.dst[nb] = D.dtab[mt].as<Occ12>() + pm.tab_off[mt];
+        a.n[nb] = (int)pm.pre[mt].size();
+        a.n_tab[nb] = (unsigned)D.dense_n[mt];
+        most = std::max(most, a.n[nb]);
+        nb++;
+        D.dense_built++;
+      }
+      if (D.dense_used[mt] > from) HIP_TRY(c, hipMemsetAsync(D.dtab[mt].as<Occ12>() + from, 0xff, (D.dense_used[mt] - from) * sizeof(Occ12), st));
+    }
+    if (nb > 0 && most > 0) {
+      hipLaunchKernelGGL(occ_dense_build_kernel, dim3((unsigned)std::min(64, (most + kBlock - 1) / kBlock), (unsigned)nb), dim3(kBlock), 0, st, a);
+      HIP_TRY(c, hipGetLastError());
+    }
+  }
+  for (int mt = 0; mt < 2; mt++) {
+    const Occ12* base = D.dtab[mt].as<Occ12>();
+    DenseMate& v = D.dense_view[mt];
+    v.A = base + s.planner.memo(ids[0]).tab_off[mt];
+    v.B = ids.size() > 1 ? base + s.planner.memo(ids[1]).tab_off[mt] : base;
+    v.n = (unsigned)D.dense_n[mt]; v.pad_ = 0;
+  }
+  return 0;
+}
+
 const Occ12* occdev_table(const PairedSet& s, int mt) { return s.occdev.tab[mt][s.occdev.serial & 1].as<Occ12>(); }
 
 void paired_images_refresh(PairedSet& s) {
diff --git a/gaml_amd/csrc/paired_launch.hip.h b/gaml_amd/csrc/paired_launch.hip.h
--- a/gaml_amd/csrc/paired_launch.hip.h
+++ b/gaml_amd/csrc/paired_launch.hip.h
@@ -89,8 +89,10 @@
   s.planner.finish(s.mate);
   PairedSet::OccDev& D = s.occdev;
   D.taken = device_route && occdev_route_ok(c, s);
+  D.dense = D.taken && occdense_route_ok(c, s);
   size_t up_bytes = 0;
-  if (D.taken) { if (int e = occdev_launch(c, s, st, &up_bytes)) return e; }
+  if (D.dense) { if (int e = occdense_prepare(c, s, st, &up_bytes)) return e; }
+  else if (D.taken) { if (int e = occdev_launch(c, s, st, &up_bytes)) return e; }
   c->prof[6] = (double)up_bytes;
   const double q1 = now_us();
   const bool cov = s.cfg.penalty_constant > 0;
@@ -101,6 +103,7 @@
   s.planner.apply(s.mate, s.image, !D.taken, D.image_stale);
   D.image_stale = D.taken;
   if (D.taken) D.dev_calls++; else D.host_calls++;
+  if (D.dense) D.dense_calls++;
   p.assembled_records = s.planner.assembled(0) + s.planner.assembled(1);
   p.general = !D.taken && (!s.image[0].general_wids.empty() || !s.image[1].general_wids.empty());
   if (trace) fprintf(stderr, "pass2: finish %.1f us, starts %.1f us, images %.1f us\n", q1 - q0, q2 - q1, now_us() - q2);
@@ -436,13 +439,14 @@
   const char* arena = nullptr;
   SetDev sd;
   s.occdev.check_dup = s.occdev.taken;
+  s.occdev.last_dense = s.occdev.dense;
   if (s.occdev.taken) {
     PairedLayout Lt;
     Lt.tfloor_off = s.persist.off_tfloor;
     paired_pack_thresholds(s, Lt, (double)(2 * tl), (char*)s.persist.dev);
     _mm_sfence();
     paired_persist_view(s, total_len, sd);
-    for (int mt = 0; mt < 2; mt++) sd.occ12[mt] = occdev_table(s, mt);
+    for (int mt = 0; mt < 2; mt++) sd.occ12[mt] = s.occdev.dense ? s.occdev.dense_view[mt].A : occdev_table(s, mt);
     c->prof[6] += 256.0 * sizeof(double);
   } else if (resident) {
     if (int e = paired_persist_update(c, s, (double)(2 * tl), st, &p, cov ? &L : nullptr)) return e;
@@ -484,6 +488,8 @@
   s.last_host_partials = c->host_results;
   s.last_sets = 1;
   paired_apply_set(a, sd);
+  const bool dense = s.occdev.taken && s.occdev.dense;
+  if (dense) { a.dense[0] = s.occdev.dense_view[0]; a.dense[1] = s.occdev.dense_view[1]; a.dup = (int*)s.occdev.dup.dev; }
   a.out = out4;
   a.timeline = nullptr;
   const bool timeline = KNOB(c, 3) == 8;
@@ -504,12 +510,14 @@
     s.last_total_blocks = n_partials;
     const dim3 grid(a.total_blocks), block(kBlock);
     hipEvent_t e0 = ev ? ev->first : nullptr, e1 = ev ? ev->second : nullptr;
+    if (dense && (fin_mode != 2 || gen_set || cov || timeline)) return fail(c, GAML_HIP_ESTATE, "dense occurrence route outside its conditions");
 #define GAML_LAUNCH_SCORE(...) hipExtLaunchKernelGGL((paired_score_kernel<__VA_ARGS__>), grid, block, KNOB(c, 1), st, e0, e1, 0, a)
 #ifdef GAML_HIP_DEV
     if (timeline) GAML_LAUNCH_SCORE(false, false, true);
     else
 #endif
-    if (gen_set) { if (fin_mode) GAML_LAUNCH_SCORE(false, true); else GAML_LAUNCH_SCORE(true, true); }
+    if (dense) GAML_LAUNCH_SCORE(false, false, false, false, true);
+    else if (gen_set) { if (fin_mode) GAML_LAUNCH_SCORE(false, true); else GAML_LAUNCH_SCORE(true, true); }
     else if (cov && a.memo && KNOB(c, 21) == 0) { if (fin_mode) GAML_LAUNCH_SCORE(false, false, false, true); else GAML_LAUNCH_SCORE(true, false, false, true); }
     else if (fin_mode) GAML_LAUNCH_SCORE(false, false);
     else GAML_LAUNCH_SCORE(true, false);
diff --git a/include/gaml_hip_debug.h b/include/gaml_hip_debug.h
--- a/include/gaml_hip_debug.h
+++ b/include/gaml_hip_debug.h
@@ -30,6 +30,7 @@
 int32_t gaml_hip_debug_block_partials(gaml_hip_ctx* ctx, int readset, int32_t set, double* sums, int32_t* zeros, int32_t cap, int32_t* layout8);
 
 int gaml_hip_debug_occ_route(gaml_hip_ctx* ctx, int readset, int64_t* out6);
+int gaml_hip_debug_occ_dense(gaml_hip_ctx* ctx, int readset, int64_t* out8);
 int gaml_hip_debug_occ_check(gaml_hip_ctx* ctx, int readset, int64_t* out4);
 
 int32_t gaml_hip_debug_batch_bad_bases(gaml_hip_ctx* ctx, int readset, int64_t* out, int32_t cap);
```
